# toposware/schnorr-sig

Measured on AMD Instinct MI355X. Metric: Schnorr verifications/sec, 2^20-sig batch, 1/2/4/8 MI355X; bit-exact vs CPU, higher is better.
Workload: dtype u64

## Files before the change

include/schnorr_sig_amd.h:

```cpp
#ifndef SCHNORR_SIG_AMD_H
#define SCHNORR_SIG_AMD_H

#include <stddef.h>
#include <stdint.h>

#ifdef __cplusplus
extern "C" {
#endif

#define SSA_SIGNATURE_LENGTH 81
#define SSA_AFFINE_PK_LENGTH 96
#define SSA_SCALAR_LENGTH 32
#define SSA_PUBLIC_KEY_LENGTH 49
#define SSA_DIGEST_LENGTH 32
#define SSA_PARAMS_LENGTH 2816

#define SSA_OK 0
#define SSA_INVALID_PUBLIC_KEY 1
#define SSA_INVALID_SIGNATURE 2
#define SSA_MALFORMED 3

#define SSA_ERR_ARG (-1)
#define SSA_ERR_HIP (-2)
#define SSA_ERR_PARAMS (-3)
// ... 393 lines not shown
int ssa_aggregator_push(ssa_ctx *ctx, ssa_aggregator *ag, const uint8_t *sigs, const uint8_t *pks, const uint8_t *pk_inf,
                        const uint8_t *msgs, const uint64_t *msg_off, size_t msg_stride, size_t msg_len, size_t n,
                        uint32_t flags, uint8_t *status_out, uint64_t *n_kept_out);
int ssa_aggregator_push_device(ssa_ctx *ctx, ssa_aggregator *ag, const uint8_t *d_sigs, const uint8_t *d_pks,
                               const uint8_t *d_pk_inf, const uint8_t *d_msgs, const uint64_t *d_msg_off, size_t msg_stride,
                               size_t msg_len, size_t n, uint32_t flags, uint8_t *d_status_out, uint64_t *n_kept_out);
int ssa_aggregator_push_cached(ssa_ctx *ctx, ssa_aggregator *ag, ssa_keycache *kc, const uint8_t *sigs, const uint8_t *pks,
                               const uint8_t *pk_inf, const uint8_t *msgs, const uint64_t *msg_off, size_t msg_stride,
                               size_t msg_len, size_t n, uint8_t *status_out, uint64_t *n_kept_out, uint64_t stats_out[12]);
int ssa_aggregator_push_cached_device(ssa_ctx *ctx, ssa_aggregator *ag, ssa_keycache *kc, const uint8_t *d_sigs,
                                      const uint8_t *d_pks, const uint8_t *d_pk_inf, const uint8_t *d_msgs,
                                      const uint64_t *d_msg_off, size_t msg_stride, size_t msg_len, size_t n,
                                      uint8_t *d_status_out, uint64_t *n_kept_out, uint64_t stats_out[12]);
int ssa_aggregator_push_keyed_cached(ssa_ctx *ctx, ssa_aggregator *ag, ssa_keycache *kc, const uint8_t *keyed,
                                     const uint8_t *msgs, const uint64_t *msg_off, size_t msg_stride, size_t msg_len,
                                     size_t n, uint8_t *status_out, uint64_t *n_kept_out, uint64_t stats_out[12]);
int ssa_aggregator_push_keyed_cached_device(ssa_ctx *ctx, ssa_aggregator *ag, ssa_keycache *kc, const uint8_t *d_keyed,
                                            const uint8_t *d_msgs, const uint64_t *d_msg_off, size_t msg_stride,
                                            size_t msg_len, size_t n, uint8_t *d_status_out, uint64_t *n_kept_out,
                                            uint64_t stats_out[12]);
int ssa_aggregator_finish(ssa_ctx *ctx, ssa_aggregator *ag, size_t n_take, uint8_t *agg_out);
int ssa_aggregator_finish_device(ssa_ctx *ctx, ssa_aggregator *ag, size_t n_take, uint8_t *d_agg_out);
int ssa_aggregator_keys(ssa_ctx *ctx, ssa_aggregator *ag, size_t n_take, uint8_t *keys49_out);
int ssa_aggregator_keys_device(ssa_ctx *ctx, ssa_aggregator *ag, size_t n_take, uint8_t *d_keys49_out);
int ssa_debug_aggregator_bytes(size_t capacity, size_t block_lanes, uint32_t flags, uint64_t out[5]);
int ssa_debug_aggregator_plan(uint64_t held, uint64_t m, uint64_t block_lanes, uint64_t out[4]);
int ssa_aggregator_drop_front(ssa_ctx *ctx, ssa_aggregator *ag, size_t n);
int ssa_aggregator_remove(ssa_ctx *ctx, ssa_aggregator *ag, const uint8_t *drop, size_t n_bytes, uint64_t *n_kept_out);
int ssa_aggregator_remove_device(ssa_ctx *ctx, ssa_aggregator *ag, const uint8_t *d_drop, size_t n_bytes,
                                 uint64_t *n_kept_out);
int ssa_aggregator_finish_select(ssa_ctx *ctx, ssa_aggregator *ag, const uint32_t *order, size_t m, uint8_t *agg_out,
                                 uint8_t *keys49_out);
int ssa_aggregator_finish_select_device(ssa_ctx *ctx, ssa_aggregator *ag, const uint32_t *d_order, size_t m,
                                        uint8_t *d_agg_out, uint8_t *d_keys49_out, uint32_t *d_result_out);
int ssa_aggregator_remove_indices(ssa_ctx *ctx, ssa_aggregator *ag, const uint32_t *order, size_t m, uint64_t *n_kept_out);
int ssa_aggregator_remove_indices_device(ssa_ctx *ctx, ssa_aggregator *ag, const uint32_t *d_order, size_t m,
                                         uint64_t *n_kept_out);
int ssa_debug_aggregator_remove_plan(uint64_t held, uint64_t first_changed, uint64_t new_held, uint64_t block_lanes,
                                     uint64_t out[4]);

typedef struct ssa_aggverifier ssa_aggverifier;
int ssa_aggverifier_create(ssa_ctx *ctx, size_t capacity, size_t block_lanes, uint32_t flags, ssa_aggverifier **out);
void ssa_aggverifier_destroy(ssa_aggverifier *av);
int ssa_aggverifier_reset(ssa_aggverifier *av);
int ssa_aggverifier_info(ssa_aggverifier *av, uint64_t out[8]);
int ssa_aggverifier_push(ssa_ctx *ctx, ssa_aggverifier *av, const uint8_t *rs49, const uint8_t *pks, const uint8_t *pk_inf,
                         const uint8_t *msgs, const uint64_t *msg_off, size_t msg_stride, size_t msg_len, size_t n);
int ssa_aggverifier_push_device(ssa_ctx *ctx, ssa_aggverifier *av, const uint8_t *d_rs49, const uint8_t *d_pks,
                                const uint8_t *d_pk_inf, const uint8_t *d_msgs, const uint64_t *d_msg_off,
                                size_t msg_stride, size_t msg_len, size_t n);
int ssa_aggverifier_finish(ssa_ctx *ctx, ssa_aggverifier *av, const uint8_t *e_agg32, size_t n_take);
int ssa_aggverifier_finish_device(ssa_ctx *ctx, ssa_aggverifier *av, const uint8_t *d_e_agg, size_t n_take,
                                  uint32_t *d_verdict_out);
int ssa_debug_aggverifier_record(ssa_ctx *ctx, ssa_aggverifier *av, size_t n_take, uint64_t *d_record24_out);
int ssa_aggverifier_push_cached(ssa_ctx *ctx, ssa_aggverifier *av, ssa_keycache *kc, const uint8_t *rs49, const uint8_t *pks,
                                const uint8_t *pk_inf, const uint8_t *msgs, const uint64_t *msg_off, size_t msg_stride,
                                size_t msg_len, size_t n, uint64_t stats_out[8]);
int ssa_aggverifier_push_cached_device(ssa_ctx *ctx, ssa_aggverifier *av, ssa_keycache *kc, const uint8_t *d_rs49,
                                       const uint8_t *d_pks, const uint8_t *d_pk_inf, const uint8_t *d_msgs,
                                       const uint64_t *d_msg_off, size_t msg_stride, size_t msg_len, size_t n,
                                       uint64_t stats_out[8]);
int ssa_aggverifier_push_cached_wire(ssa_ctx *ctx, ssa_aggverifier *av, ssa_keycache *kc, const uint8_t *rs49,
                                     const uint8_t *pks49, const uint8_t *msgs, const uint64_t *msg_off, size_t msg_stride,
                                     size_t msg_len, size_t n, uint64_t stats_out[8]);
int ssa_aggverifier_push_cached_wire_device(ssa_ctx *ctx, ssa_aggverifier *av, ssa_keycache *kc, const uint8_t *d_rs49,
                                            const uint8_t *d_pks49, const uint8_t *d_msgs, const uint64_t *d_msg_off,
                                            size_t msg_stride, size_t msg_len, size_t n, uint64_t stats_out[8]);
size_t ssa_debug_aggverifier_key_span(void);

#define SSA_ABI_VERSION 5
int ssa_abi_version(void);

int ssa_debug_arith(ssa_ctx *ctx, int op, const uint64_t *a, const uint64_t *b, size_t n,
                    size_t a_stride, size_t b_stride, uint64_t *out, size_t out_stride);
int ssa_debug_fault_after_chunk(ssa_ctx *ctx, int chunk);
int ssa_debug_poison_workspaces(ssa_ctx *ctx, int byte);
int ssa_debug_table_read(ssa_ctx *ctx, int which, uint64_t first_row, uint64_t n, uint64_t *rows_out);
int ssa_debug_table_xor(ssa_ctx *ctx, int which, uint64_t row, uint32_t word, uint64_t mask);
int ssa_debug_corrupt_table_builds(int n);
int ssa_debug_keytab_xor(ssa_keyset *ks, ssa_keycache *kc, int what, uint64_t key, uint32_t word, uint64_t mask);
int ssa_debug_keytab_read(ssa_keyset *ks, ssa_keycache *kc, int what, uint64_t key, uint64_t *words_out);
int ssa_debug_tail_plan(unsigned waves, unsigned pieces, unsigned gens, int uniform, unsigned min_main, size_t n,
                        uint32_t flags, uint32_t out[14]);
int ssa_debug_screen_plan(size_t n, uint32_t coeff_bytes, uint64_t out[8]);
int ssa_debug_screen_segments(ssa_ctx *ctx, uint32_t k);
int ssa_debug_dedup_device(ssa_ctx *ctx, const uint8_t *d_pks, const uint8_t *d_pk_inf, size_t n,
                           uint32_t *d_key_idx_out, uint64_t out[2]);
int ssa_debug_dedup_config(ssa_ctx *ctx, double max_distinct_ratio, uint32_t probe_bound);
int ssa_debug_keycache_plan(uint64_t capacity, uint64_t held, uint64_t u, uint64_t m, uint32_t *plan_out);
int ssa_debug_keycache_keep(uint64_t capacity, uint64_t u, uint64_t m, const uint64_t hist[64], uint64_t out[2]);
int ssa_debug_chacha20(ssa_ctx *ctx, const uint8_t key[32], const uint8_t nonce[12], uint32_t counter0,
                       size_t n_blocks, uint8_t *out);
int ssa_bench_fpmul(ssa_ctx *ctx, int variant, double *fpmul_per_s);

#ifdef __cplusplus
}
#endif
#endif
```

schnorr-sig_amd/__init__.py:

```python
import ctypes as C
import os

import numpy as np

_HERE = os.path.dirname(os.path.abspath(__file__))
LIB_PATH = os.environ.get("SSA_LIB") or os.path.join(_HERE, "csrc", "libschnorr_sig_amd.so")

SCALAR_LENGTH = 32
PRIVATE_KEY_LENGTH = 32
BASEFIELD_LENGTH = 48
PUBLIC_KEY_LENGTH = 49
AFFINE_PUBLIC_KEY_LENGTH = 96
KEY_PAIR_LENGTH = 32
SIGNATURE_LENGTH = 81
KEYED_SIGNATURE_LENGTH = 130

OK, INVALID_PUBLIC_KEY, INVALID_SIGNATURE, MALFORMED = 0, 1, 2, 3
ERR_ARG, ERR_HIP, ERR_PARAMS, ERR_NO_DEVICE, ERR_TABLE = -1, -2, -3, -4, -5
TABLE_COMB, TABLE_CT = 0, 1
SELFCHECK_FIELDS = ("rows", "bad", "first_bad", "ctab_rows", "ctab_bad", "ctab_first_bad", "builds", "bits")
FLAG_CHECK_TORSION = 1
FLAG_FORCE_LANE = 2
FLAG_FORCE_COOP = 4
FLAG_SIG_FLAG_BYTE = 8
# ... 58 lines not shown
        return
    import importlib.util
    spec = importlib.util.find_spec("torch")
    if spec is None or not spec.submodule_search_locations:
        HIP_RUNTIME_BOUND = "system runtime (torch is not installed)"
        return
    path = os.path.join(list(spec.submodule_search_locations)[0], "lib", "libamdhip64.so")
    if not os.path.exists(path):
        HIP_RUNTIME_BOUND = "system runtime (torch carries no libamdhip64.so)"
        return
    try:
        C.CDLL(path, mode=C.RTLD_GLOBAL)
        HIP_RUNTIME_BOUND = path
    except OSError as exc:
        import warnings
        HIP_RUNTIME_BOUND = "system runtime (torch's copy did not load: %s)" % exc
        warnings.warn("schnorr_sig_amd: torch's HIP runtime %s did not load (%s); importing torch later in this process "
                      "will bring a second runtime" % (path, exc))


def _load():
    if not os.path.exists(LIB_PATH):
        raise ImportError(
            "schnorr_sig_amd: HIP library %s is missing; run `python -c 'import __graft_entry__ as g; "
            "g.build()'` (hipcc --offload-arch=gfx950). There is no CPU fallback." % LIB_PATH)
    _share_hip_runtime_with_torch()
    lib = C.CDLL(LIB_PATH)
    vp, sz, u32, u64p, i32 = C.c_void_p, C.c_size_t, C.c_uint32, C.POINTER(C.c_uint64), C.c_int
    sigs = {
        "ssa_ctx_create": (i32, [C.POINTER(vp), i32, vp, sz]),
        "ssa_ctx_create_ex": (i32, [C.POINTER(vp), i32, vp, sz, u32, C.c_uint64]),
        "ssa_ctx_info": (i32, [vp, u64p]),
        "ssa_pubkey_many": (i32, [vp, vp, sz, vp]),
        "ssa_pubkey_many_device": (i32, [vp, vp, sz, vp]),
        "ssa_ctx_destroy": (None, [vp]),
        "ssa_strerror": (C.c_char_p, [i32]),
        "ssa_default_params": (vp, []),
        "ssa_ctx_set_stream": (i32, [vp, vp]),
        "ssa_ctx_uses_default_params": (i32, [vp]),
        "ssa_ctx_sync": (i32, [vp]),
        "ssa_ctx_enable_timing": (i32, [vp, i32]),
        "ssa_ctx_read_timing": (i32, [vp, C.c_char_p, C.POINTER(C.c_double), u64p]),
        "ssa_verify": (i32, [vp, vp, vp, vp, sz, u32]),
        "ssa_verify_many": (i32, [vp, vp, vp, vp, vp, vp, sz, sz, sz, u32, vp, u64p]),
        "ssa_verify_batch": (i32, [vp, vp, vp, vp, vp, vp, sz, sz, sz, u32]),
        "ssa_hash_message_many": (i32, [vp, vp, vp, vp, vp, sz, sz, sz, vp]),
        "ssa_rescue_hash_many": (i32, [vp, vp, u32, sz, vp]),
        "ssa_keygen_sign_many": (i32, [vp, vp, vp, vp, vp, sz, sz, sz, vp, vp]),
        "ssa_verify_many_device": (i32, [vp, vp, vp, vp, vp, vp, sz, sz, sz, u32, vp, vp]),
        "ssa_hash_message_many_device": (i32, [vp, vp, vp, vp, vp, sz, sz, sz, vp]),
        "ssa_rescue_hash_many_device": (i32, [vp, vp, u32, sz, vp]),
        "ssa_keygen_sign_many_device": (i32, [vp, vp, vp, vp, vp, sz, sz, sz, vp, vp]),
        "ssa_verify_batch_msm": (i32, [vp, vp, vp, vp, vp, vp, sz, sz, sz, vp]),
        "ssa_verify_batch_msm_device": (i32, [vp, vp, vp, vp, vp, vp, sz, sz, sz, vp, u32, vp]),
        "ssa_verify_keyed_many": (i32, [vp, vp, vp, vp, sz, sz, sz, u32, vp, u64p]),
        "ssa_keyset_create": (i32, [vp, vp, vp, sz, u32, C.POINTER(vp)]),
        "ssa_keyset_create_device": (i32, [vp, vp, vp, sz, u32, C.POINTER(vp)]),
        "ssa_keyset_destroy": (None, [vp]),
        "ssa_keyset_status": (i32, [vp, vp]),
        "ssa_verify_many_indexed": (i32, [vp, vp, vp, vp, vp, vp, sz, sz, sz, u32, vp, u64p]),
        "ssa_verify_many_indexed_device": (i32, [vp, vp, vp, vp, vp, vp, sz, sz, sz, u32, vp, vp]),
        "ssa_multi_create": (i32, [C.POINTER(vp), C.POINTER(i32), i32, vp, sz]),
        "ssa_multi_destroy": (None, [vp]),
        "ssa_multi_verify_many": (i32, [vp, vp, vp, vp, vp, vp, sz, sz, sz, u32, vp, u64p]),
        "ssa_multi_verify_batch_msm": (i32, [vp, vp, vp, vp, vp, vp, sz, sz, sz, vp]),
        "ssa_decompress_many": (i32, [vp, vp, sz, vp, vp, vp]),
        "ssa_decompress_many_device": (i32, [vp, vp, sz, vp, vp, vp]),
        "ssa_debug_arith": (i32, [vp, i32, vp, vp, sz, sz, sz, vp, sz]),
        "ssa_bench_fpmul": (i32, [vp, i32, C.POINTER(C.c_double)]),
        "ssa_debug_chacha20": (i32, [vp, vp, vp, u32, sz, vp]),
        "ssa_verify_batch_msm_partial_device": (i32, [vp, vp, vp, vp, vp, vp, sz, sz, sz, vp, u32, vp]),
        "ssa_verify_batch_msm_partial": (i32, [vp, vp, vp, vp, vp, vp, sz, sz, sz, vp, vp]),
        "ssa_msm_combine_device": (i32, [vp, vp, sz, vp]),
        "ssa_msm_combine": (i32, [vp, vp, sz]),
        "ssa_abi_version": (i32, []),
        "ssa_keygen_sign_many_ex": (i32, [vp, vp, vp, vp, vp, sz, sz, sz, u32, vp, vp]),
        "ssa_keygen_sign_many_ex_device": (i32, [vp, vp, vp, vp, vp, sz, sz, sz, u32, vp, vp]),
        "ssa_compress_many": (i32, [vp, vp, vp, sz, vp, vp]),
        "ssa_compress_many_device": (i32, [vp, vp, vp, sz, vp, vp]),
        "ssa_ctx_stream_release": (i32, [vp, vp]),
        "ssa_ctx_stream_acquire": (i32, [vp, vp]),
        "ssa_debug_fault_after_chunk": (i32, [vp, i32]),
        "ssa_debug_tail_plan": (i32, [u32, u32, u32, i32, u32, sz, u32, vp]),
        "ssa_verify_batch_screened": (i32, [vp, vp, vp, vp, vp, vp, sz, sz, sz, vp, vp, u64p]),
        "ssa_verify_batch_screened_device": (i32, [vp, vp, vp, vp, vp, vp, sz, sz, sz, vp, u32, vp, vp]),
        "ssa_debug_screen_plan": (i32, [sz, u32, vp]),
        "ssa_debug_screen_segments": (i32, [vp, u32]),
        "ssa_verify_many_dedup": (i32, [vp, vp, vp, vp, vp, vp, sz, sz, sz, u32, vp, u64p, vp]),
        "ssa_verify_many_dedup_device": (i32, [vp, vp, vp, vp, vp, vp, sz, sz, sz, u32, vp, vp, vp]),
        "ssa_verify_many_screened": (i32, [vp, vp, vp, vp, vp, vp, sz, sz, sz, u32, vp, vp, u64p, vp]),
        "ssa_verify_many_screened_device": (i32, [vp, vp, vp, vp, vp, vp, sz, sz, sz, u32, vp, u32, vp, vp, vp]),
        "ssa_keycache_create": (i32, [vp, sz, C.POINTER(vp)]),
        "ssa_keycache_destroy": (None, [vp]),
        "ssa_keycache_clear": (i32, [vp]),
        "ssa_keycache_info": (i32, [vp, u64p]),
        "ssa_verify_many_cached": (i32, [vp, vp, vp, vp, vp, vp, vp, sz, sz, sz, u32, vp, vp, u64p, vp]),
        "ssa_verify_many_cached_device": (i32, [vp, vp, vp, vp, vp, vp, vp, sz, sz, sz, u32, vp, u32, vp, vp, vp]),
        "ssa_keycache_create_ex": (i32, [vp, sz, u32, C.POINTER(vp)]),
        "ssa_verify_keyed_many_cached": (i32, [vp, vp, vp, vp, vp, sz, sz, sz, u32, vp, vp, u64p, vp]),
        "ssa_verify_keyed_many_cached_device": (i32, [vp, vp, vp, vp, vp, sz, sz, sz, u32, vp, u32, vp, vp, vp]),
        "ssa_verify_keyed_many_device": (i32, [vp, vp, vp, vp, sz, sz, sz, u32, vp, vp]),
        "ssa_debug_keycache_plan": (i32, [C.c_uint64, C.c_uint64, C.c_uint64, C.c_uint64, C.POINTER(u32)]),
        "ssa_keycache_set_eviction": (i32, [vp, u32]),
        "ssa_keycache_eviction_info": (i32, [vp, u64p]),
        "ssa_debug_keycache_keep": (i32, [C.c_uint64, C.c_uint64, C.c_uint64, u64p, u64p]),
        "ssa_debug_dedup_device": (i32, [vp, vp, vp, sz, vp, vp]),
        "ssa_debug_dedup_config": (i32, [vp, C.c_double, u32]),
        "ssa_xprv_master_many": (i32, [vp, vp, sz, vp, vp]),
        "ssa_xprv_master_many_device": (i32, [vp, vp, sz, vp, vp]),
        "ssa_xprv_derive_many": (i32, [vp, vp, sz, vp, vp, sz, u32, vp, vp]),
        "ssa_xprv_derive_many_device": (i32, [vp, vp, sz, vp, vp, sz, u32, vp, vp]),
        "ssa_xpub_derive_many": (i32, [vp, vp, sz, vp, vp, sz, vp, vp, vp, vp]),
        "ssa_xpub_derive_many_device": (i32, [vp, vp, sz, vp, vp, sz, vp, vp, vp, vp]),
        "ssa_debug_hmac_sha512": (i32, [vp, vp, sz, vp, sz, sz, vp]),
        "ssa_signer_set_create": (i32, [vp, vp, sz, C.POINTER(vp)]),
        "ssa_signer_set_create_device": (i32, [vp, vp, sz, sz, C.POINTER(vp)]),
        "ssa_signer_set_destroy": (None, [vp]),
        "ssa_signer_set_status": (i32, [vp, vp]),
        "ssa_signer_set_public_keys": (i32, [vp, vp, vp]),
        "ssa_sign_many_indexed": (i32, [vp, vp, vp, vp, vp, vp, sz, sz, sz, u32, vp]),
        "ssa_sign_many_indexed_device": (i32, [vp, vp, vp, vp, vp, vp, sz, sz, sz, u32, vp, vp]),
        "ssa_ctx_selfcheck": (i32, [vp, u32, u64p]),
        "ssa_debug_table_read": (i32, [vp, i32, C.c_uint64, C.c_uint64, vp]),
        "ssa_debug_table_xor": (i32, [vp, i32, C.c_uint64, u32, C.c_uint64]),
        "ssa_debug_corrupt_table_builds": (i32, [i32]),
        "ssa_keyset_selfcheck": (i32, [vp, u32, vp, u64p]),
        "ssa_keycache_selfcheck": (i32, [vp, u32, u64p]),
        "ssa_debug_keytab_xor": (i32, [vp, vp, i32, C.c_uint64, u32, C.c_uint64]),
        "ssa_debug_keytab_read": (i32, [vp, vp, i32, C.c_uint64, vp]),
        "ssa_keygen_sign_many_rng": (i32, [vp, vp, vp, vp, sz, sz, sz, u32, vp, vp]),
        "ssa_keygen_sign_many_rng_device": (i32, [vp, vp, vp, vp, sz, sz, sz, u32, vp, vp]),
        "ssa_sign_many_indexed_rng": (i32, [vp, vp, vp, vp, vp, sz, sz, sz, u32, vp]),
        "ssa_sign_many_indexed_rng_device": (i32, [vp, vp, vp, vp, vp, sz, sz, sz, u32, vp, vp]),
        "ssa_signer_set_generate": (i32, [vp, sz, C.POINTER(vp)]),
        "ssa_signer_set_secret_keys": (i32, [vp, vp]),
        "ssa_debug_pin_rng": (i32, [vp, vp]),
        "ssa_debug_draw_scalars": (i32, [vp, vp, sz, vp]),
        "ssa_debug_poison_workspaces": (i32, [vp, i32]),
        "ssa_aggregate_many": (i32, [vp, vp, vp, vp, vp, vp, sz, sz, sz, u32, vp, vp, u64p]),
        "ssa_aggregate_many_device": (i32, [vp, vp, vp, vp, vp, vp, sz, sz, sz, u32, vp, vp, vp]),
        "ssa_verify_aggregate": (i32, [vp, vp, vp, vp, vp, vp, sz, sz, sz]),
        "ssa_verify_aggregate_device": (i32, [vp, vp, vp, vp, vp, vp, sz, sz, sz, vp]),
        "ssa_debug_aggregate_coeffs": (i32, [vp, vp, vp, vp, vp, vp, sz, sz, sz, vp]),
        "ssa_aggregate_shard_tops_device": (i32, [vp, vp, u32, vp, vp, vp, sz, sz, sz, sz, vp, vp]),
        "ssa_aggregate_root_device": (i32, [vp, vp, sz, sz, sz, vp]),
        "ssa_aggregate_shard_fold_device": (i32, [vp, vp, vp, vp, sz, sz, vp, vp, vp, vp, vp]),
        "ssa_verify_aggregate_shard_device": (i32, [vp, vp, vp, vp, vp, vp, sz, sz, vp, sz, sz, vp, vp]),
        "ssa_aggregate_combine_device": (i32, [vp, vp, sz, vp]),
        "ssa_verify_aggregate_combine_device": (i32, [vp, vp, sz, vp, sz, vp]),
        "ssa_aggregate_many_sliced": (i32, [vp, vp, vp, vp, vp, vp, sz, sz, sz, u32, vp, vp, u64p]),
        "ssa_aggregate_many_sliced_device": (i32, [vp, vp, vp, vp, vp, vp, sz, sz, sz, u32, vp, vp, vp]),
        "ssa_verify_aggregate_sliced": (i32, [vp, vp, vp, vp, vp, vp, sz, sz, sz]),
        "ssa_verify_aggregate_sliced_device": (i32, [vp, vp, vp, vp, vp, vp, sz, sz, sz, vp]),
        "ssa_multi_aggregate_many": (i32, [vp, vp, vp, vp, vp, vp, sz, sz, sz, u32, vp, vp, u64p]),
        "ssa_multi_verify_aggregate": (i32, [vp, vp, vp, vp, vp, vp, sz, sz, sz]),
        "ssa_debug_aggregate_shard_coeffs": (i32, [vp, vp, sz, sz, vp]),
        "ssa_aggregate_valid_many": (i32, [vp, vp, vp, vp, vp, vp, sz, sz, sz, vp, vp, u64p, vp]),
        "ssa_aggregate_valid_many_device": (i32, [vp, vp, vp, vp, vp, vp, sz, sz, sz, vp, vp, u64p, vp]),
        "ssa_aggregate_valid_many_cached": (i32, [vp, vp, vp, vp, vp, vp, vp, sz, sz, sz, vp, vp, u64p, vp, vp, vp, vp]),
        "ssa_aggregate_valid_many_cached_device": (i32, [vp, vp, vp, vp, vp, vp, vp, sz, sz, sz, vp, vp, u64p, vp, vp, vp,
                                                         vp]),
        "ssa_aggregate_valid_keyed_many_cached": (i32, [vp, vp, vp, vp, vp, sz, sz, sz, vp, vp, u64p, vp, vp, vp]),
        "ssa_aggregate_valid_keyed_many_cached_device": (i32, [vp, vp, vp, vp, vp, sz, sz, sz, vp, vp, u64p, vp, vp, vp]),
        "ssa_debug_aggregate_keep": (i32, [vp, vp, sz, vp, u64p]),
        "ssa_verify_aggregates_many": (i32, [vp, vp, u64p, sz, vp, vp, vp, vp, sz, sz, vp]),
        "ssa_verify_aggregates_many_device": (i32, [vp, vp, u64p, sz, vp, vp, vp, vp, sz, sz, vp]),
# ... 1024 lines not shown
        seed = _np_u8(bytearray(seed44))
        if seed.size != 44:
            raise ValueError("the seed is 44 bytes")
        _check(_lib.ssa_debug_pin_rng(self._ctx, _ptr(seed)), "ssa_debug_pin_rng")

    def debug_draw_scalars(self, blocks):
        b = _np_u8(blocks, 128)
        out = np.zeros((b.shape[0], 32), dtype=np.uint8)
        _check(_lib.ssa_debug_draw_scalars(self._ctx, _ptr(b), b.shape[0], _ptr(out)), "ssa_debug_draw_scalars")
        return out

    def set_stream(self, hip_stream):
        _check(_lib.ssa_ctx_set_stream(self._ctx, C.c_void_p(hip_stream or 0)), "ssa_ctx_set_stream")

    def sync(self):
        _check(_lib.ssa_ctx_sync(self._ctx), "ssa_ctx_sync")

    def stream_release(self, consumer_stream):
        _check(_lib.ssa_ctx_stream_release(self._ctx, C.c_void_p(consumer_stream or 0)), "ssa_ctx_stream_release")

    def stream_acquire(self, producer_stream):
        _check(_lib.ssa_ctx_stream_acquire(self._ctx, C.c_void_p(producer_stream or 0)), "ssa_ctx_stream_acquire")

    def selfcheck(self):
        out = (C.c_uint64 * 8)()
        rc = _lib.ssa_ctx_selfcheck(self._ctx, 0, out)
        if rc != ERR_TABLE:
            _check(rc, "ssa_ctx_selfcheck")
        res = dict(zip(SELFCHECK_FIELDS, (int(v) for v in out)))
        res["ok"] = rc == OK
        return res

    def debug_table_read(self, which, first_row, n):
        out = np.zeros((n, 12), dtype=np.uint64)
        _check(_lib.ssa_debug_table_read(self._ctx, int(which), int(first_row), int(n), _ptr(out)), "ssa_debug_table_read")
        return out

    def debug_table_xor(self, which, row, word, mask):
        _check(_lib.ssa_debug_table_xor(self._ctx, int(which), int(row), int(word), C.c_uint64(int(mask))),
               "ssa_debug_table_xor")

    def debug_fault_after_chunk(self, chunk):
        _check(_lib.ssa_debug_fault_after_chunk(self._ctx, int(chunk)), "ssa_debug_fault_after_chunk")

    def debug_poison_workspaces(self, byte):
        _check(_lib.ssa_debug_poison_workspaces(self._ctx, int(byte)), "ssa_debug_poison_workspaces")

    def verify_many_device(self, d_sigs, d_pks, d_msgs, n, msg_len, d_status, d_nfail, msg_stride=None,
                           d_offsets=0, d_pk_inf=0, check_torsion=False, mode=None, sig_flag_byte=False):
        _check(_lib.ssa_verify_many_device(
            self._ctx, d_sigs, d_pks, *self._dev_batch(d_pk_inf, d_msgs, d_offsets, msg_stride, msg_len, n),
            self._verify_flags(check_torsion, sig_flag_byte, mode), d_status, d_nfail), "ssa_verify_many_device")

    def keygen_sign_many_device(self, d_sks, d_nonces, d_msgs, n, msg_len, d_pks, d_sigs, msg_stride=None,
                                d_offsets=0, constant_time=False, keyed=False):
        flags = (FLAG_SIGN_CT if constant_time else 0) | (FLAG_SIGN_KEYED if keyed else 0)
        _check(_lib.ssa_keygen_sign_many_ex_device(self._ctx, d_sks, d_nonces, d_msgs, d_offsets or None,
                                                   msg_stride if msg_stride is not None else msg_len, msg_len, n, flags,
                                                   d_pks or None, d_sigs), "ssa_keygen_sign_many_ex_device")

    def compress_many_device(self, d_pks, n, d_out, d_pk_inf=0, d_status=0):
        _check(_lib.ssa_compress_many_device(self._ctx, d_pks, d_pk_inf or None, n, d_out, d_status or None),
               "ssa_compress_many_device")

    def rescue_hash_many_device(self, d_felts, per_row, n, d_out):
        _check(_lib.ssa_rescue_hash_many_device(self._ctx, d_felts, per_row, n, d_out),
               "ssa_rescue_hash_many_device")

    def hash_message_many_device(self, d_sigs, d_pks, d_msgs, n, msg_len, d_out, msg_stride=None, d_offsets=0):
        _check(_lib.ssa_hash_message_many_device(self._ctx, d_sigs, d_pks, d_msgs, d_offsets or None,
                                                 msg_stride if msg_stride is not None else msg_len, msg_len, n,
                                                 d_out), "ssa_hash_message_many_device")

    def enable_timing(self, on=True):
        _check(_lib.ssa_ctx_enable_timing(self._ctx, int(on)), "ssa_ctx_enable_timing")

    def read_timing(self, kernel):
        avg = C.c_double(0)
        cnt = C.c_uint64(0)
        _check(_lib.ssa_ctx_read_timing(self._ctx, kernel.encode(), C.byref(avg), C.byref(cnt)),
               "ssa_ctx_read_timing")
        return avg.value, int(cnt.value)

    def host_path_probe(self, sigs_t, pks_t, msgs_t, n, reps=3):
        import time
        hs, hp, hm = (t[:n].cpu().numpy() for t in (sigs_t, pks_t, msgs_t))
        st, nf = self.verify_many(hs, hp, hm, check_torsion=False, mode="lane", sig_flag_byte=True)
        t0 = time.perf_counter()
        for _ in range(reps):
            st, nf = self.verify_many(hs, hp, hm, check_torsion=False, mode="lane", sig_flag_byte=True)
        dt = (time.perf_counter() - t0) / reps
        verdict = self.verify_batch_msm(hs, hp, hm)
        t0 = time.perf_counter()
        for _ in range(reps):
            verdict = self.verify_batch_msm(hs, hp, hm)
        dt_msm = (time.perf_counter() - t0) / reps
        return {"entry_point": "ssa_verify_many (host buffers in pageable memory, copied through the library's page-locked "
                               "bounce buffers, uploads in chunks overlapped with the hash kernel)",
                "ms_per_batch": dt * 1e3, "verifications_per_sec": n / dt, "rejected": int(nf),
                "verify_batch_msm_ms_per_batch": dt_msm * 1e3, "verify_batch_msm_signatures_per_sec": n / dt_msm,
                "verify_batch_msm_verdict": int(verdict)}

    def debug_arith(self, op, a, b, out_cols):
        a = np.ascontiguousarray(a, dtype=np.uint64)
        b = np.ascontiguousarray(b, dtype=np.uint64) if b is not None else None
        n = a.shape[0]
        out = np.zeros((n, out_cols), dtype=np.uint64)
        _check(_lib.ssa_debug_arith(self._ctx, op, _ptr(a), _ptr(b), n, a.shape[1],
                                    b.shape[1] if b is not None else 0, _ptr(out), out_cols), "ssa_debug_arith")
        return out

    def bench_fpmul(self, variant):
        v = C.c_double(0)
        _check(_lib.ssa_bench_fpmul(self._ctx, variant, C.byref(v)), "ssa_bench_fpmul")
        return v.value


def debug_corrupt_table_builds(n):
    _check(_lib.ssa_debug_corrupt_table_builds(int(n)), "ssa_debug_corrupt_table_builds")


KEYCHECK_DEEP, KEYCHECK_REPAIR = 1, 2
KEYCHECK_FIELDS = ("keys_checked", "keys_bad", "first_bad_key", "ladder_entries_checked", "comb_rows_checked",
                   "keys_rebuilt_and_compared", "combs_skipped", "rows_repaired")
KEYTAB_LADDER, KEYTAB_STATUS, KEYTAB_KEY, KEYTAB_PK_INF, KEYTAB_COMB = 0, 1, 2, 3, 4
KEYTAB_WIRE = 5
_KEYTAB_READ_WORDS = {KEYTAB_LADDER: 512, KEYTAB_STATUS: 1, KEYTAB_KEY: 12, KEYTAB_PK_INF: 1, KEYTAB_COMB: 24,
                      KEYTAB_WIRE: 7}
KEYCACHE_WIRE = 1
KEYCACHE_EVICT = {"clear": 0, "recent": 1}


def _keycheck_result(rc, out, what):
    if rc != ERR_TABLE:
        _check(rc, what)
    res = dict(zip(KEYCHECK_FIELDS, (int(v) for v in out)))
    res["ok"] = rc == OK
    return res


class _KeyTables:

    def _pair(self):
        raise NotImplementedError

    def debug_keytab_xor(self, what, key, word, mask):
        ks, kc = self._pair()
        _check(_lib.ssa_debug_keytab_xor(ks, kc, int(what), int(key), int(word), C.c_uint64(int(mask))),
               "ssa_debug_keytab_xor")

    def debug_keytab_read(self, what, key):
        ks, kc = self._pair()
        out = np.zeros(_KEYTAB_READ_WORDS[int(what)], dtype=np.uint64)
        _check(_lib.ssa_debug_keytab_read(ks, kc, int(what), int(key), _ptr(out)), "ssa_debug_keytab_read")
        return out


class KeySet(_KeyTables):

    def __init__(self, engine, handle, m):
        self.engine = engine
        self.handle = handle
        self.m = int(m)

    def _pair(self):
        return self.handle, None
# ... 507 lines not shown

class MultiEngine:

    def __init__(self, devices, params=None):
        self._m = C.c_void_p()
        devs = (C.c_int * len(devices))(*[int(d) for d in devices])
        blob = (C.c_uint8 * len(params)).from_buffer_copy(bytes(params)) if params is not None else None
        _check(_lib.ssa_multi_create(C.byref(self._m), devs, len(devices), blob, len(params) if params else 0),
               "ssa_multi_create")

    def close(self):
        if self._m:
            _lib.ssa_multi_destroy(self._m)
            self._m = C.c_void_p()

    def __del__(self):
        try:
            self.close()
        except Exception:
            pass

    def verify_many(self, sigs, pks, msgs, offsets=None, check_torsion=True, pk_inf=None):
        sigs, pks = _np_u8(sigs, 81), _np_u8(pks, 96)
        n = sigs.shape[0]
        m = _np_u8(msgs)
        off = np.ascontiguousarray(offsets, dtype=np.uint64) if offsets is not None else None
        stride = mlen = 0 if off is not None else m.shape[1]
        inf = _np_u8(pk_inf) if pk_inf is not None else None
        status = np.full(n, 255, dtype=np.uint8)
        nfail = C.c_uint64(0)
        _check(_lib.ssa_multi_verify_many(self._m, _ptr(sigs), _ptr(pks), _ptr(inf), _ptr(m), _ptr(off), stride, mlen,
                                          n, FLAG_CHECK_TORSION if check_torsion else 0, _ptr(status),
                                          C.byref(nfail)), "ssa_multi_verify_many")
        return status, int(nfail.value)


    def verify_batch_msm(self, sigs, pks, msgs, offsets=None, coeffs=None, pk_inf=None):
        sigs, pks = _np_u8(sigs, 81), _np_u8(pks, 96)
        n = sigs.shape[0]
        m = _np_u8(msgs)
        off = np.ascontiguousarray(offsets, dtype=np.uint64) if offsets is not None else None
        stride = mlen = 0 if off is not None else m.shape[1]
        inf = _np_u8(pk_inf) if pk_inf is not None else None
        c = _np_u8(coeffs, 32) if coeffs is not None else None
        return _check(_lib.ssa_multi_verify_batch_msm(self._m, _ptr(sigs), _ptr(pks), _ptr(inf), _ptr(m), _ptr(off),
                                                      stride, mlen, n, _ptr(c)), "ssa_multi_verify_batch_msm")


    _msg_args = Engine._msg_args
    _agg_batch = Engine._agg_batch

    def aggregate(self, sigs, pks, msgs, offsets=None, pk_inf=None, check=False):
        n, batch, keep = self._agg_batch(sigs, 81, pks, msgs, offsets, pk_inf)
        agg = np.full(49 * n + 32, 255, dtype=np.uint8)
        status = np.full(n, 255, dtype=np.uint8)
        nfail = C.c_uint64(0)
        st = _check(_lib.ssa_multi_aggregate_many(self._m, *batch, AGG_CHECK if check else 0, _ptr(agg),
                                                  _ptr(status) if n else None, C.byref(nfail)), "ssa_multi_aggregate_many")
        return st, agg, status, int(nfail.value)

    def verify_aggregate(self, agg, pks, msgs, offsets=None, pk_inf=None):
        n, batch, keep = self._agg_batch(agg, 49, pks, msgs, offsets, pk_inf)
        if keep[0].size != 49 * n + 32:
            raise MalformedInput("an aggregate of n signatures is 49 n + 32 bytes")
        return _check(_lib.ssa_multi_verify_aggregate(self._m, *batch), "ssa_multi_verify_aggregate")

    aggregate_sliced, verify_aggregate_sliced = aggregate, verify_aggregate


_default_engine = None


def debug_tail_plan(waves, n, check_torsion=False, pieces=5, gens=1, uniform=False, min_main=0):
    out = np.zeros(14, dtype=np.uint32)
    flags = 1 if check_torsion else 0
    _check(_lib.ssa_debug_tail_plan(int(waves), int(pieces), int(gens), int(bool(uniform)), int(min_main), int(n), flags,
                                    out.ctypes.data), "ssa_debug_tail_plan")

    def dec(d):
        d = int(d)
        return (d & 1, bool(d & 2), bool(d & 4), (d >> 8) & 0xff, (d >> 16) & 0xff)
    return {"n_pieces": int(out[0]), "tail_groups": int(out[1]), "main_blocks": int(out[2]), "grid_blocks": int(out[3]),
            "pieces": [dec(out[4 + k]) for k in range(int(out[0]))], "whole": [dec(out[12]), dec(out[13])]}


def debug_screen_plan(n, coeff_bytes=0):
    out = np.zeros(8, dtype=np.uint64)
    _check(_lib.ssa_debug_screen_plan(int(n), int(coeff_bytes), out.ctypes.data), "ssa_debug_screen_plan")
    keys = ("segments", "segment_lanes", "window_bits", "windows", "r_windows", "buckets_per_window", "slices",
            "total_segments")
    return {k: int(v) for k, v in zip(keys, out)}


def debug_aggregates_plan(counts, msm_slice=1 << 23, small_max=3072):
    counts = np.ascontiguousarray(counts, dtype=np.uint64)
    cp = counts.ctypes.data_as(C.POINTER(C.c_uint64)) if counts.size else None
    need = _lib.ssa_debug_aggregates_plan(cp, counts.size, int(msm_slice), int(small_max), None, 0)
    if need < 0:
        return None
    out = np.zeros(need, dtype=np.uint64)
    _check(_lib.ssa_debug_aggregates_plan(cp, counts.size, int(msm_slice), int(small_max),
                                          out.ctypes.data_as(C.POINTER(C.c_uint64)), need), "ssa_debug_aggregates_plan")
    w = [int(v) for v in out]
    keys = ("first_aggregate", "aggregates", "first_lane", "lanes", "segment_lanes", "bucket")
    groups = [dict(zip(keys, w[4 + 6 * g:10 + 6 * g])) for g in range(w[2])]
    pos, passes = 4 + 6 * w[2], []
    for _ in range(w[1]):
        cnt = w[pos]
        passes.append([tuple(w[pos + 1 + 4 * d:pos + 5 + 4 * d]) for d in range(cnt)])
        pos += 1 + 4 * cnt
    return {"lanes": w[0], "groups": groups, "passes": passes, "descriptors": w[3]}


def debug_aggregates_fold_plan(counts):
    counts = np.ascontiguousarray(counts, dtype=np.uint64)
    cp = counts.ctypes.data_as(C.POINTER(C.c_uint64)) if counts.size else None
    need = _lib.ssa_debug_aggregates_fold_plan(cp, counts.size, None, 0)
    if need < 0:
        return None
    out = np.zeros(need, dtype=np.uint64)
    _check(_lib.ssa_debug_aggregates_fold_plan(cp, counts.size, out.ctypes.data_as(C.POINTER(C.c_uint64)), need),
           "ssa_debug_aggregates_fold_plan")
    return int(out[0]), out[1:]


def default_engine():
    global _default_engine
    if _default_engine is None:
        _default_engine = Engine(0)
    return _default_engine


class PublicKey:

    def __init__(self, affine96, is_identity=False):
        b = bytes(affine96)
        if len(b) != AFFINE_PUBLIC_KEY_LENGTH:
            raise ValueError("PublicKey needs 96 bytes of affine coordinates")
        self.affine = b
        self.is_identity = bool(is_identity)

    def verify_signature(self, signature, message):
        return signature.verify(message, self)

    @classmethod
    def from_private(cls, sk, engine=None):
        return KeyPair.from_private(sk, engine).public_key

    @classmethod
    def from_bytes(cls, b49, engine=None):
        b = bytes(b49)
        if len(b) != PUBLIC_KEY_LENGTH:
            raise ValueError("compressed public key needs 49 bytes")
        pks, inf, st = (engine or default_engine()).decompress_many(np.frombuffer(b, np.uint8))
        if st[0] != 0:
            return None
        return cls(pks[0].tobytes(), is_identity=bool(inf[0]))

    def to_bytes(self, engine=None):
        out, st = (engine or default_engine()).compress_many(np.frombuffer(self.affine, np.uint8),
                                                             pk_inf=np.array([1 if self.is_identity else 0], np.uint8))
        if st[0] != OK:
            raise MalformedInput("PublicKey holds a non-canonical limb")
        return out[0].tobytes()

    def __eq__(self, o):
# ... 544 lines not shown
```

schnorr-sig_amd/csrc/ssa_api.hip:

```cpp
#define SSA_KERNELS_DEFINE 1
#include "ssa_ctx.hpp"
#include "ssa_keycache.hpp"
#include "ssa_keyed.hpp"
#include "ssa_aggregate.hpp"
#include "ssa_aggcache.hpp"
#include "ssa_aggregator.hpp"
#include "ssa_aggverifier.hpp"

#include <sys/random.h>

#include <atomic>
#include <climits>
#include <functional>
#include <initializer_list>
#include <memory>
#include <mutex>
#include <thread>

static const unsigned char k_default_params[SSA_PARAMS_LENGTH] = {
#include "../params/params_default.inc"
};

extern "C" const char *ssa_strerror(int rc) {
    switch (rc) {
        case SSA_OK: return "ok";
        case SSA_INVALID_PUBLIC_KEY: return "The public key is not an element of the prime subgroup.";
        case SSA_INVALID_SIGNATURE: return "The signature is invalid or was incorrectly computed.";
        case SSA_MALFORMED: return "malformed input (the reference would panic)";
        case SSA_ERR_ARG: return "invalid argument";
        case SSA_ERR_HIP: return "HIP runtime error";
        case SSA_ERR_PARAMS: return "invalid parameter blob";
        case SSA_ERR_NO_DEVICE: return "no HIP device";
        case SSA_ERR_TABLE: return "a precomputed table failed its self-check";
        default: return "unknown";
    }
}

extern "C" const void *ssa_default_params(void) { return k_default_params; }

extern "C" int ssa_abi_version(void) { return SSA_ABI_VERSION; }

struct SharedGtab {
    int device = 0;
    u32 bits = 0;
    u64 gen[12] = {};
    u64 *d_gtab = nullptr;
    int refs = 0;
    int builds = 0;
    bool retired = false;
};
static std::mutex g_gtab_mu;
static std::vector<SharedGtab *> g_gtabs;

static inline size_t gtab_bytes(u32 bits) { return gtab_entries(bits) * 12 * sizeof(u64); }

static std::atomic<int> g_corrupt_builds{0};

static int debug_corrupt_build(ssa_ctx *ctx, SharedGtab *g) {
    int n = g_corrupt_builds.load();
    while (n > 0 && !g_corrupt_builds.compare_exchange_weak(n, n - 1)) {
    }
    if (n <= 0) return 0;
    u64 *p = g->d_gtab + 12 * (((size_t)(gtab_windows(g->bits) / 2) << g->bits) + 12345) + 7, v = 0;
    HIP_TRY(hipMemcpyAsync(&v, p, sizeof v, hipMemcpyDeviceToHost, ctx->stream));
    HIP_TRY(hipStreamSynchronize(ctx->stream));
    v ^= 1ull << 17;
    HIP_TRY(hipMemcpyAsync(p, &v, sizeof v, hipMemcpyHostToDevice, ctx->stream));
    HIP_TRY(hipStreamSynchronize(ctx->stream));
    return 0;
}

static SharedGtab *gtab_acquire(ssa_ctx *ctx, const DevParams &hp, u32 bits, bool *bad_table) {
    std::lock_guard<std::mutex> lock(g_gtab_mu);
    u64 gen[12];
    for (int i = 0; i < 6; i++) {
        gen[i] = hp.gen_x[i];
        gen[6 + i] = hp.gen_y[i];
    }
    for (SharedGtab *g : g_gtabs)
        if (g->device == ctx->device && g->bits == bits && std::memcmp(g->gen, gen, sizeof gen) == 0) {
            g->refs++;
            return g;
        }
    SharedGtab *g = new SharedGtab();
    g->device = ctx->device;
    g->bits = bits;
    std::memcpy(g->gen, gen, sizeof gen);
    void *gbase = nullptr;
    bool ok = hipMalloc((void **)&g->d_gtab, gtab_bytes(bits)) == hipSuccess &&
              hipMalloc(&gbase, gbase_entries(bits) * 12 * sizeof(u64)) == hipSuccess;
    if (ok) {
        bool clean = false;
        for (int b = 0; b < 2 && ok && !clean; b++) {
            hipLaunchKernelGGL(ssa_k_gbase, dim3(grid_for(gbase_entries(bits), 256)), dim3(256), 0, ctx->stream,
                               ctx->d_params, (u64 *)gbase, bits);
            hipLaunchKernelGGL(ssa_k_gtable, dim3(grid_for(gtab_entries(bits) / 8, 256)), dim3(256), 0, ctx->stream,
                               (const u64 *)gbase, g->d_gtab, bits);
            g->builds++;
            ok = hipGetLastError() == hipSuccess && hipStreamSynchronize(ctx->stream) == hipSuccess &&
                 debug_corrupt_build(ctx, g) == 0;
            uint64_t res[2] = {0, 0};
            ok = ok && ssa_internal_gtab_check(ctx, g->d_gtab, bits, res) == 0;
            clean = ok && res[0] == 0;
        }
        if (ok && !clean) {
            *bad_table = true;
            ok = false;
        }
    } else {
        (void)hipGetLastError();
    }
    if (gbase) (void)hipFree(gbase);
    if (!ok) {
        if (g->d_gtab) (void)hipFree(g->d_gtab);
        delete g;
        return nullptr;
    }
    g->refs = 1;
    g_gtabs.push_back(g);
    return g;
}

static void gtab_release(SharedGtab *g) {
    if (!g) return;
    std::lock_guard<std::mutex> lock(g_gtab_mu);
    if (--g->refs > 0) return;
    forget_handle(g_gtabs, g);
    (void)hipSetDevice(g->device);
    (void)hipFree(g->d_gtab);
    delete g;
}

static int validate_params(const DevParams &p) {
    if (std::memcmp(p.magic, "SSAPARM1", 8) != 0) return SSA_ERR_PARAMS;
    if (p.n_rounds == 0 || p.n_rounds > 8) return SSA_ERR_PARAMS;
    if (p.rate_off != 0 && p.rate_off != 4) return SSA_ERR_PARAMS;
    if (p.cap_len_idx < -1 || p.cap_len_idx > 11) return SSA_ERR_PARAMS;
    if (p.pad_mode > 1 || p.digest_off > 8) return SSA_ERR_PARAMS;
    for (int i = 0; i < 144; i++)
        if (p.mds[i] >= FP_P) return SSA_ERR_PARAMS;
    for (int i = 0; i < 96; i++)
        if (p.ark1[i] >= FP_P || p.ark2[i] >= FP_P) return SSA_ERR_PARAMS;
    for (int i = 0; i < 6; i++)
        if (p.gen_x[i] >= FP_P || p.gen_y[i] >= FP_P) return SSA_ERR_PARAMS;
    return 0;
}

template <class T>
static bool env_u64(const char *name, uint64_t lo, uint64_t hi, T &knob) {
    const char *e = std::getenv(name);
    const uint64_t v = e ? std::strtoull(e, nullptr, 10) : 0;
    if (!e || v < lo || v > hi) return false;
    knob = (T)v;
    return true;
}
template <class T>
static bool env_int(const char *name, int lo, int hi, T &knob) {
    const char *e = std::getenv(name);
    const int v = e ? std::atoi(e) : 0;
    if (!e || v < lo || v > hi) return false;
    knob = (T)v;
    return true;
}
template <class T>
static void env_one_of(const char *name, std::initializer_list<int> set, T &knob) {
    int v = 0;
    if (env_int(name, INT_MIN, INT_MAX, v) && std::find(set.begin(), set.end(), v) != set.end()) knob = (T)v;
}
static void env_flag(const char *name, bool &knob) {
    int v = 0;
    if (env_int(name, INT_MIN, INT_MAX, v)) knob = v != 0;
}

static void ctx_read_env(ssa_ctx *ctx, uint32_t *gtab_bits, uint64_t *hbm_budget_bytes) {
    CtxKnobs &k = ctx->knobs;
    if (env_u64("SSA_COOP_MAX_N", 0, UINT64_MAX, k.coop_max_n)) k.coop_max_n_torsion = k.coop_max_n;
    env_u64("SSA_MSM_SMALL_MAX", 0, UINT64_MAX, k.msm_small_max);
    env_one_of("SSA_VERIFY_BLOCK", {64, 128, 256}, k.verify_block);
    env_u64("SSA_LANE_SLICE", 256, UINT64_MAX, k.lane_slice);
    env_u64("SSA_MSM_SLICE", 256, (uint64_t)1 << 23, k.msm_slice);
    env_u64("SSA_AGG_BLOCK", 1, (uint64_t)1 << 30, k.agg_block);
    env_int("SSA_MSM_TREE_GROUP", 2, 64, k.msm_tree_group);
    env_int("SSA_TAIL_PIECES", 0, VP_MAX, k.tail_pieces);
    env_int("SSA_TAIL_GENS", 1, 8, k.tail_gens);
    env_flag("SSA_TAIL_UNIFORM", k.tail_uniform);
    env_int("SSA_TAIL_MIN_MAIN", INT_MIN, INT_MAX, k.tail_min_main);
    env_flag("SSA_TAIL_REVERSED", k.tail_reversed);
    env_int("SSA_TAIL_WAVES", INT_MIN, INT_MAX, k.tail_waves_override);
    env_flag("SSA_MSM_OVERLAP", k.msm_overlap);
    env_int("SSA_PIPELINE_CHUNKS", 1, 8, k.pipeline_chunks);
    env_flag("SSA_TWO_STREAMS", ctx->two_streams);
    uint64_t mb = 0;
    if (*hbm_budget_bytes == 0 && env_u64("SSA_HBM_BUDGET_MB", 0, UINT64_MAX, mb)) *hbm_budget_bytes = mb << 20;
    if (*gtab_bits == 0) env_one_of("SSA_GTAB_BITS", {16, 20, 22, 24}, *gtab_bits);
}

static int ctx_create(ssa_ctx **out, int device, const void *params, size_t params_len, uint32_t gtab_bits,
                      uint64_t hbm_budget_bytes, const CtxKnobs *inherit) {
    if (!out) return SSA_ERR_ARG;
    *out = nullptr;
    if (gtab_bits != 0 && gtab_bits != 16 && gtab_bits != 20 && gtab_bits != 22 && gtab_bits != 24) return SSA_ERR_ARG;
    int count = 0;
    if (hipGetDeviceCount(&count) != hipSuccess || count == 0) return SSA_ERR_NO_DEVICE;
    if (device < 0 || device >= count) return SSA_ERR_ARG;
    DevParams hp;
    if (params) {
        if (params_len != sizeof(DevParams)) return SSA_ERR_PARAMS;
        std::memcpy(&hp, params, sizeof hp);
    } else {
        std::memcpy(&hp, k_default_params, sizeof hp);
    }
    const bool is_default = std::memcmp(&hp, k_default_params, sizeof hp) == 0;
    if (int rc = validate_params(hp)) return rc;
    hp.flags = 0;
    bool small_mds = true;
    for (int i = 0; i < 144; i++) small_mds = small_mds && hp.mds[i] <= 0xffffffffull;
    if (small_mds) hp.flags |= PRM_FLAG_SMALL_MDS;
    bool tiny_mds = true;
    for (int i = 0; i < 144; i++) tiny_mds = tiny_mds && hp.mds[i] < 0x10000ull;
    if (tiny_mds) hp.flags |= PRM_FLAG_TINY_MDS;
    HIP_TRY(hipSetDevice(device));
    std::unique_ptr<ssa_ctx, decltype(&ssa_ctx_destroy)> guard(new ssa_ctx(), ssa_ctx_destroy);
    ssa_ctx *ctx = guard.get();
    ctx->device = device;
    ctx->default_params = is_default;
    if (inherit) ctx->knobs = *inherit;
    else ctx_read_env(ctx, &gtab_bits, &hbm_budget_bytes);
    HIP_TRY(hipStreamCreateWithFlags(&ctx->own_stream, hipStreamNonBlocking));
    HIP_TRY(hipStreamCreateWithFlags(&ctx->copy_stream, hipStreamNonBlocking));
    for (auto &st : ctx->hash_stream) HIP_TRY(hipStreamCreateWithFlags(&st, hipStreamNonBlocking));
    HIP_TRY(hipEventCreateWithFlags(&ctx->pipe_start, hipEventDisableTiming));
    HIP_TRY(hipEventCreateWithFlags(&ctx->order_ev, hipEventDisableTiming));
    for (int i = 0; i < 8; i++) {
        HIP_TRY(hipEventCreateWithFlags(&ctx->copy_done[i], hipEventDisableTiming));
        HIP_TRY(hipEventCreateWithFlags(&ctx->hash_done[i], hipEventDisableTiming));
    }
    ctx->stream = ctx->own_stream;
    if (!inherit) {
        hipDeviceProp_t prop;
        int occ = 0;
        if (hipGetDeviceProperties(&prop, device) == hipSuccess &&
            hipOccupancyMaxActiveBlocksPerMultiprocessor(&occ, ssa_k_verify, 256, 0) == hipSuccess && occ > 0)
            ctx->knobs.verify_waves = (unsigned)prop.multiProcessorCount * (unsigned)occ * 4u;
        (void)hipGetLastError();
        if (ctx->knobs.tail_waves_override) ctx->knobs.verify_waves = ctx->knobs.tail_waves_override;
    }
    HIP_TRY(hipMalloc((void **)&ctx->d_params, sizeof(DevParams)));
    HIP_TRY(hipMemcpy(ctx->d_params, &hp, sizeof hp, hipMemcpyHostToDevice));
    ctx->h_params = hp;
    if (hbm_budget_bytes == 0) {
        size_t free_b = 0, total_b = 0;
        if (hipMemGetInfo(&free_b, &total_b) != hipSuccess) free_b = 0;
        hbm_budget_bytes = free_b / 10;
    }
    ctx->hbm_budget = hbm_budget_bytes;
    static const u32 k_widths[4] = {24, 22, 20, 16};
    bool bad_table = false;
    for (u32 wbits : k_widths) {
        if (gtab_bits ? wbits > gtab_bits : (wbits > 16 && gtab_bytes(wbits) > hbm_budget_bytes)) continue;
        ctx->gtab_share = gtab_acquire(ctx, hp, wbits, &bad_table);
        if (ctx->gtab_share) break;
    }
    if (!ctx->gtab_share) return bad_table ? SSA_ERR_TABLE : SSA_ERR_HIP;
    if (ctx->ws_fail.reserve(64)) return SSA_ERR_HIP;
    ctx->d_gtab = ctx->gtab_share->d_gtab;
    ctx->gtab_bits = ctx->gtab_share->bits;
    unsigned gen_ok = 0;
    hipLaunchKernelGGL(ssa_k_check_generator, dim3(1), dim3(64), 0, ctx->stream, ctx->d_params,
                       (const u64 *)ctx->d_gtab, (unsigned *)ctx->ws_fail.p);
    HIP_TRY(hipGetLastError());
    HIP_TRY(hipMemcpyAsync(&gen_ok, ctx->ws_fail.p, sizeof gen_ok, hipMemcpyDeviceToHost, ctx->stream));
    HIP_TRY(hipStreamSynchronize(ctx->stream));
    if (gen_ok != 1u) return SSA_ERR_PARAMS;
    *out = guard.release();
    return 0;
}

extern "C" int ssa_ctx_create_ex(ssa_ctx **out, int device, const void *params, size_t params_len, uint32_t gtab_bits,
                                 uint64_t hbm_budget_bytes) {
    return ctx_create(out, device, params, params_len, gtab_bits, hbm_budget_bytes, nullptr);
}

extern "C" int ssa_ctx_create(ssa_ctx **out, int device, const void *params, size_t params_len) {
    return ssa_ctx_create_ex(out, device, params, params_len, 0u, 0ull);
}

ssa_ctx *ssa_internal_twin(ssa_ctx *ctx) {
    if (ctx->is_twin || !ctx->two_streams) return nullptr;
    if (!ctx->twin) {
        DevParams hp = ctx->h_params;
        hp.flags = 0;
        if (ctx_create(&ctx->twin, ctx->device, &hp, sizeof hp, ctx->gtab_bits, ctx->hbm_budget, &ctx->knobs) != 0) {
            ctx->two_streams = false;
            return nullptr;
        }
        ctx->twin->is_twin = true;
    }
    ctx->twin->knobs = ctx->knobs;
    return ctx->twin;
}

template <class T, class F>
static void orphan_handles(std::vector<T *> &v, F &&release) {
    for (T *h : v) {
        release(h);
        h->ctx = nullptr;
    }
    v.clear();
}

extern "C" void ssa_ctx_destroy(ssa_ctx *ctx) {
    if (!ctx) return;
    (void)hipSetDevice(ctx->device);
    if (ctx->stream) (void)hipStreamSynchronize(ctx->stream);
    if (ctx->twin) {
        ssa_ctx_destroy(ctx->twin);
        ctx->twin = nullptr;
    }
    orphan_handles(ctx->keysets, [](ssa_keyset *ks) { ks->release_all(); });
    orphan_handles(ctx->signer_sets, [](ssa_signer_set *ss) { ss->wipe_release(); });
    orphan_handles(ctx->keycaches, [](ssa_keycache *kc) { kc->release_all(); });
    orphan_handles(ctx->aggregators, [](ssa_aggregator *ag) { agx_release_all(*ag); });
    orphan_handles(ctx->aggverifiers, [](ssa_aggverifier *av) { agx_release_all(*av); });
    for (auto &kv : ctx->timed)
        for (auto &t : kv.second) {
            (void)hipEventDestroy(t.start);
            (void)hipEventDestroy(t.stop);
        }
    for_each_devbuf(ctx, [](DevBuf &b) { b.release(); });
    for_each_hostbuf(ctx, [](HostBuf &b) { b.release(); });
    if (ctx->d_params) (void)hipFree(ctx->d_params);
    gtab_release(ctx->gtab_share);
    ctx->gtab_share = nullptr;
    ctx->d_gtab = nullptr;
    for (auto &ev : ctx->copy_done)
        if (ev) (void)hipEventDestroy(ev);
    for (auto &ev : ctx->hash_done)
        if (ev) (void)hipEventDestroy(ev);
    if (ctx->pipe_start) (void)hipEventDestroy(ctx->pipe_start);
    if (ctx->order_ev) (void)hipEventDestroy(ctx->order_ev);
    if (ctx->agm_plan_ev) (void)hipEventDestroy(ctx->agm_plan_ev);
    for (auto &st : ctx->hash_stream)
        if (st) (void)hipStreamDestroy(st);
    if (ctx->copy_stream) (void)hipStreamDestroy(ctx->copy_stream);
    if (ctx->own_stream) (void)hipStreamDestroy(ctx->own_stream);
    delete ctx;
}

extern "C" int ssa_ctx_info(const ssa_ctx *ctx, uint64_t out[8]) {
    if (!ctx || !out) return SSA_ERR_ARG;
    auto reserved = [](const ssa_ctx *c) {
        uint64_t sum = 0;
        for_each_devbuf(c, [&](const DevBuf &b) { sum += b.cap; });
        return sum;
    };
    out[0] = ctx->gtab_bits;
    out[1] = gtab_windows(ctx->gtab_bits);
    out[2] = gtab_bytes(ctx->gtab_bits);
    out[3] = reserved(ctx) + (ctx->twin ? reserved(ctx->twin) : 0);
    out[4] = ctx->knobs.lane_slice;
    out[5] = ctx->knobs.msm_slice;
    out[6] = ctx->hbm_budget;
    out[7] = ctx->two_streams && !ctx->is_twin ? 1 : 0;
    return 0;
}

extern "C" int ssa_ctx_selfcheck(ssa_ctx *ctx, uint32_t flags, uint64_t out[8]) {
    if (!ctx || !out || flags != 0) return SSA_ERR_ARG;
    HIP_TRY(hipSetDevice(ctx->device));
    uint64_t g[2], c[3] = {0, 0, ~0ull};
    if (int rc = ssa_internal_gtab_check(ctx, ctx->d_gtab, ctx->gtab_bits, g)) return rc;
    if (g[0] == 0)
        if (int rc = ssa_internal_ctab_selfcheck(ctx, c)) return rc;
    out[0] = gtab_entries(ctx->gtab_bits);
    out[1] = g[0];
    out[2] = g[1];
    out[3] = c[0];
    out[4] = c[1];
    out[5] = c[2];
    out[6] = (uint64_t)ctx->gtab_share->builds;
    out[7] = ctx->gtab_bits;
    if (g[0]) {
        std::lock_guard<std::mutex> lock(g_gtab_mu);
        SharedGtab *sg = ctx->gtab_share;
        if (!sg->retired) {
            sg->retired = true;
            forget_handle(g_gtabs, sg);
        }
    }
    return g[0] || c[1] ? SSA_ERR_TABLE : SSA_OK;
}

extern "C" int ssa_ctx_uses_default_params(const ssa_ctx *ctx) { return ctx ? (ctx->default_params ? 1 : 0) : SSA_ERR_ARG; }

extern "C" int ssa_ctx_set_stream(ssa_ctx *ctx, void *hip_stream) {
    if (!ctx) return SSA_ERR_ARG;
    HIP_TRY(hipStreamSynchronize(ctx->stream));
    ctx->stream = hip_stream ? (hipStream_t)hip_stream : ctx->own_stream;
    return 0;
}

extern "C" int ssa_ctx_stream_release(ssa_ctx *ctx, void *consumer_stream) {
    if (!ctx) return SSA_ERR_ARG;
    HIP_TRY(hipSetDevice(ctx->device));
    if ((hipStream_t)consumer_stream == ctx->stream) return 0;
    HIP_TRY(hipEventRecord(ctx->order_ev, ctx->stream));
    HIP_TRY(hipStreamWaitEvent((hipStream_t)consumer_stream, ctx->order_ev, 0));
    return 0;
}

extern "C" int ssa_ctx_stream_acquire(ssa_ctx *ctx, void *producer_stream) {
    if (!ctx) return SSA_ERR_ARG;
    HIP_TRY(hipSetDevice(ctx->device));
    if ((hipStream_t)producer_stream == ctx->stream) return 0;
    HIP_TRY(hipEventRecord(ctx->order_ev, (hipStream_t)producer_stream));
    HIP_TRY(hipStreamWaitEvent(ctx->stream, ctx->order_ev, 0));
    return 0;
}

extern "C" int ssa_ctx_sync(ssa_ctx *ctx) {
    if (!ctx) return SSA_ERR_ARG;
    HIP_TRY(hipStreamSynchronize(ctx->stream));
    return 0;
}

extern "C" int ssa_ctx_enable_timing(ssa_ctx *ctx, int on) {
    if (!ctx) return SSA_ERR_ARG;
    ctx->knobs.timing = on != 0;
    return 0;
}

extern "C" int ssa_ctx_read_timing(ssa_ctx *ctx, const char *kernel, double *avg_ms, uint64_t *launches) {
    if (!ctx || !kernel) return SSA_ERR_ARG;
    HIP_TRY(hipStreamSynchronize(ctx->stream));
    double total = 0;
    uint64_t cnt = 0;
    for (ssa_ctx *c : {ctx, ctx->twin}) {
        if (!c) continue;
        if (c != ctx) HIP_TRY(hipStreamSynchronize(c->stream));
        auto it = c->timed.find(kernel);
        if (it == c->timed.end()) continue;
        for (auto &t : it->second) {
            float ms = 0;
            if (hipEventElapsedTime(&ms, t.start, t.stop) == hipSuccess) {
                total += ms;
                cnt++;
            }
            (void)hipEventDestroy(t.start);
            (void)hipEventDestroy(t.stop);
        }
        c->timed.erase(it);
    }
    if (avg_ms) *avg_ms = cnt ? total / (double)cnt : 0.0;
    if (launches) *launches = cnt;
    return 0;
}

extern "C" int ssa_hash_message_many_device(ssa_ctx *ctx, const uint8_t *d_sigs, const uint8_t *d_pks,
                                            const uint8_t *d_msgs, const uint64_t *d_msg_off,
                                            size_t msg_stride, size_t msg_len, size_t n,
                                            uint8_t *d_digests_out) {
    const MsgView mv{d_msgs, d_msg_off, msg_stride, msg_len};
    if (!ctx || (n && (!d_sigs || !d_pks || !d_digests_out))) return SSA_ERR_ARG;
    if (int rc = check_msgs(mv, n)) return rc;
    if (n == 0) return 0;
    HIP_TRY(hipSetDevice(ctx->device));
    return timed_launch(ctx, "ssa_k_hash", [&] {
        hipLaunchKernelGGL(ssa_k_hash, dim3(grid_for(n, 256)), dim3(256), 0, ctx->stream, ctx->d_params,
                           d_sigs, d_pks, mv, n, (u64 *)nullptr, d_digests_out, (const u32 *)nullptr, 0u);
    });
}

extern "C" int ssa_rescue_hash_many_device(ssa_ctx *ctx, const uint64_t *d_felts, uint32_t felts_per_row,
                                           size_t n, uint64_t *d_digests_out) {
    if (!ctx || (n && (!d_digests_out || (felts_per_row && !d_felts)))) return SSA_ERR_ARG;
    if (n == 0) return 0;
    HIP_TRY(hipSetDevice(ctx->device));
    return timed_launch(ctx, "ssa_k_rescue", [&] {
        hipLaunchKernelGGL(ssa_k_rescue, dim3(grid_for(n, 256)), dim3(256), 0, ctx->stream, ctx->d_params,
                           (const u64 *)d_felts, felts_per_row, n, (u64 *)d_digests_out);
    });
}

int ssa_internal_hash_chunk(ssa_ctx *ctx, hipStream_t hs, const DevBatch &b, size_t cnt, uint64_t *d_h) {
    hipLaunchKernelGGL(ssa_k_hash, dim3(grid_for(cnt, 256)), dim3(256), 0, hs, ctx->d_params, b.sigs, b.pks, b.msgs, cnt,
                       (u64 *)d_h, (u8 *)nullptr, (const u32 *)nullptr, 0u);
    HIP_TRY(hipGetLastError());
    return 0;
}

int ssa_internal_hash_scalars(ssa_ctx *ctx, const DevBatch &b, size_t n) {
    if (ctx->ws_h.reserve(n * 4 * sizeof(u64))) return SSA_ERR_HIP;
    return timed_launch(ctx, "ssa_k_hash", [&] {
        hipLaunchKernelGGL(ssa_k_hash, dim3(grid_for(n, 256)), dim3(256), 0, ctx->stream, ctx->d_params,
                           b.sigs, b.pks, b.msgs, n, (u64 *)ctx->ws_h.p, (u8 *)nullptr, (const u32 *)nullptr, 0u);
    });
}

int ssa_internal_hash_scalars_digests(ssa_ctx *ctx, const DevBatch &b, size_t n, uint64_t *d_h, uint8_t *d_dig) {
    return timed_launch(ctx, "ssa_k_hash", [&] {
        hipLaunchKernelGGL(ssa_k_hash, dim3(grid_for(n, 256)), dim3(256), 0, ctx->stream, ctx->d_params,
                           b.sigs, b.pks, b.msgs, n, (u64 *)d_h, (u8 *)d_dig, (const u32 *)nullptr, 0u);
    });
}

struct TailKnobs {
    unsigned pieces, gens, waves, block, min_main;
    bool uniform, reversed;
};
static TailPlan tail_plan_of(const TailKnobs &kn, size_t cnt, uint32_t flags) {
    const TailKnobs *ctx = &kn;
    TailPlan tp{};
    const bool torsion = (flags & SSA_FLAG_CHECK_TORSION) != 0;
    tp.whole[0] = 0u | 2u | 4u | ((u32)LADDER_STEPS_Q << 16);
    tp.whole[1] = 1u | 2u | 4u | ((u32)LADDER_STEPS << 16);
    const u32 n_groups = (u32)((cnt + 63) / 64);
    const unsigned cap = torsion ? (unsigned)VP_MAX - 1u : (unsigned)VP_MAX;
    const unsigned want = ctx->pieces < cap ? ctx->pieces : cap;
    const u32 tail0 = ctx->gens * ctx->waves;
    if (want < 2 || ctx->block != 256 || tail0 == 0 || n_groups < tail0 + ctx->min_main * ctx->waves) return tp;
    const u32 main_groups = ((n_groups - tail0) / 4u) * 4u;
    tp.main_blocks = main_groups / 4u;
    tp.tail_groups = ((n_groups - main_groups + 3u) / 4u) * 4u;
    const double DBL = 2642.0, ADD = 3738.0, TABLE = 57000.0, TAIL = 45000.0;
    struct Step { int pass, it; double cost; };
    std::vector<Step> steps;
    for (int pass = torsion ? 0 : 1; pass < 2; pass++)
        for (int it = 0; it < (pass == 0 ? LADDER_STEPS_Q : LADDER_STEPS); it++)
            steps.push_back({pass, it, (pass == 0 ? (double)QNAF_GAP[it + 1] : 5.0) * DBL + ADD});
    double total = TABLE + TAIL;
    for (const Step &st : steps) total += st.cost;
    std::vector<double> target;
    double frac = 0.0, f = 0.5;
    for (unsigned k = 0; k + 1 < want; k++) {
        frac += ctx->uniform ? 1.0 / (double)want : f;
        if (k + 2 < want) f *= 0.5;
        target.push_back(total * frac);
    }
    std::vector<std::pair<size_t, size_t>> pieces;
    size_t cur = 0, tix = 0;
    double acc = TABLE;
    for (size_t idx = 0; idx < steps.size(); idx++) {
        bool cut = false;
        if (idx > cur) {
            if (steps[idx].pass != steps[idx - 1].pass) cut = true;
            else if (tix < target.size() && acc + steps[idx].cost * 0.5 >= target[tix]) cut = true;
        }
        if (cut) {
            pieces.push_back({cur, idx});
            cur = idx;
        }
        while (tix < target.size() && acc + steps[idx].cost * 0.5 >= target[tix]) tix++;
        acc += steps[idx].cost;
    }
    pieces.push_back({cur, steps.size()});
    if (pieces.size() < 2 || pieces.size() > (size_t)VP_MAX) return tp;
    for (const auto &pc : pieces) {
        const int pass = steps[pc.first].pass, lo = steps[pc.first].it, hi = steps[pc.second - 1].it + 1;
        const int n_steps = pass == 0 ? LADDER_STEPS_Q : LADDER_STEPS;
        tp.ph[tp.n_pieces++] = (u32)pass | (lo == 0 ? 2u : 0u) | (hi == n_steps ? 4u : 0u) | ((u32)lo << 8) | ((u32)hi << 16);
    }
    tp.reversed = ctx->reversed ? 1u : 0u;
    return tp;
}
static TailPlan tail_plan(const ssa_ctx *ctx, size_t cnt, uint32_t flags) {
    return tail_plan_of({ctx->knobs.tail_pieces, ctx->knobs.tail_gens, ctx->knobs.verify_waves, ctx->knobs.verify_block, ctx->knobs.tail_min_main,
                         ctx->knobs.tail_uniform, ctx->knobs.tail_reversed}, cnt, flags);
}

extern "C" int ssa_debug_tail_plan(unsigned waves, unsigned pieces, unsigned gens, int uniform, unsigned min_main, size_t n,
                                   uint32_t flags, uint32_t out[14]) {
    if (!out) return SSA_ERR_ARG;
    const TailPlan tp = tail_plan_of({pieces, gens, waves, 256u, min_main, uniform != 0, false}, n, flags);
    out[0] = tp.n_pieces;
    out[1] = tp.tail_groups;
    out[2] = tp.main_blocks;
    out[3] = tp.n_pieces ? tail_grid_blocks(tp) : (uint32_t)((n + 255) / 256);
    for (int k = 0; k < VP_MAX; k++) out[4 + k] = tp.ph[k];
    out[12] = tp.whole[0];
    out[13] = tp.whole[1];
    return 0;
}

static int verify_slices(ssa_ctx *ctx, const DevBatch &b, const u64 *d_h, size_t n, uint32_t flags, uint8_t *d_status_out,
                         unsigned long long *d_fail) {
    return for_dev_slices(b, n, ctx->knobs.lane_slice, [&](size_t lo, size_t cnt, const DevBatch &s) {
        const TailPlan tp = tail_plan(ctx, cnt, flags);
        unsigned blocks = grid_for(cnt, ctx->knobs.verify_block);
        if (tp.n_pieces) {
            if (ctx->tail_done.reserve(2 * (size_t)tp.tail_groups * sizeof(u32)) ||
                ctx->tail_park.reserve((size_t)tp.tail_groups * PARK_WORDS * 64 * sizeof(u64)))
                return SSA_ERR_HIP;
            HIP_TRY(hipMemsetAsync(ctx->tail_done.p, 0, 2 * (size_t)tp.tail_groups * sizeof(u32), ctx->stream));
            blocks = tail_grid_blocks(tp);
        }
        return timed_launch(ctx, "ssa_k_verify", [&] {
            hipLaunchKernelGGL(ssa_k_verify, dim3(blocks), dim3(ctx->knobs.verify_block), 0,
                               ctx->stream, s.sigs, s.pks, s.pk_inf, d_h + 4 * lo, (const u64 *)ctx->d_gtab,
                               (u64 *)ctx->ws_tab.p, cnt, flags, d_status_out + lo, d_fail, tp, (u32 *)ctx->tail_done.p,
                               (u64 *)ctx->tail_park.p);
        });
    });
}

int ssa_internal_verify_hashed(ssa_ctx *ctx, const DevBatch &b, const uint64_t *d_h, size_t n, uint32_t flags,
                               uint8_t *d_status_out, unsigned long long *d_fail) {
    const size_t slice = ctx->knobs.lane_slice < n ? ctx->knobs.lane_slice : n;
    if (ctx->ws_tab.reserve(slice * (size_t)(PTAB_ENTRIES * PTAB_ENTRY_U64) * sizeof(u64))) return SSA_ERR_HIP;
    return verify_slices(ctx, b, (const u64 *)d_h, n, flags, d_status_out, d_fail);
}

static int verify_one_slice(ssa_ctx *c, const DevBatch &b, size_t cnt, uint32_t flags, uint8_t *d_status_out,
                            unsigned long long *d_fail) {
    if (c->ws_h.reserve(cnt * 4 * sizeof(u64))) return SSA_ERR_HIP;
    if (c->ws_tab.reserve(cnt * (size_t)(PTAB_ENTRIES * PTAB_ENTRY_U64) * sizeof(u64))) return SSA_ERR_HIP;
    int rc = timed_launch(c, "ssa_k_hash", [&] {
        hipLaunchKernelGGL(ssa_k_hash, dim3(grid_for(cnt, 256)), dim3(256), 0, c->stream, c->d_params, b.sigs, b.pks,
                           b.msgs, cnt, (u64 *)c->ws_h.p, (u8 *)nullptr, (const u32 *)nullptr, 0u);
    });
    if (rc) return rc;
    return verify_slices(c, b, (const u64 *)c->ws_h.p, cnt, flags, d_status_out, d_fail);
}

static int verify_launch(ssa_ctx *ctx, const DevBatch &b, size_t n, uint32_t flags, uint8_t *d_status_out,
                         unsigned long long *d_fail) {
    if (takes_coop(ctx, n, flags)) {
        return timed_launch(ctx, "ssa_k_verify_coop", [&] {
            hipLaunchKernelGGL(ssa_k_verify_coop, dim3((unsigned)n), dim3(128), 0, ctx->stream, ctx->d_params, b.sigs,
                               b.pks, b.pk_inf, b.msgs, (const u64 *)ctx->d_gtab, n, flags, d_status_out, d_fail);
        });
    }
    const size_t slice = ctx->knobs.lane_slice < n ? ctx->knobs.lane_slice : n;
    if (n <= slice) return verify_one_slice(ctx, b, n, flags, d_status_out, d_fail);
    ssa_ctx *tw = ssa_internal_twin(ctx);
    if (tw) {
        HIP_TRY(hipEventRecord(ctx->order_ev, ctx->stream));
        HIP_TRY(hipStreamWaitEvent(tw->stream, ctx->order_ev, 0));
    }
    int rc = 0;
    size_t j = 0;
    for (size_t lo = 0; lo < n && rc == 0; lo += slice, j++) {
        const size_t cnt = n - lo < slice ? n - lo : slice;
        ssa_ctx *c = (tw && (j & 1u)) ? tw : ctx;
        rc = verify_one_slice(c, b.slice(lo), cnt, flags, d_status_out + lo, d_fail);
    }
    if (tw) {
        if (hipEventRecord(tw->order_ev, tw->stream) != hipSuccess ||
            hipStreamWaitEvent(ctx->stream, tw->order_ev, 0) != hipSuccess)
            return rc ? rc : SSA_ERR_HIP;
    }
    return rc;
}

extern "C" int ssa_verify_many_device(ssa_ctx *ctx, const uint8_t *d_sigs, const uint8_t *d_pks,
                                      const uint8_t *d_pk_inf, const uint8_t *d_msgs,
                                      const uint64_t *d_msg_off, size_t msg_stride, size_t msg_len,
                                      size_t n, uint32_t flags, uint8_t *d_status_out,
                                      uint64_t *d_n_fail_out) {
    const DevBatch b{d_sigs, d_pks, d_pk_inf, {d_msgs, d_msg_off, msg_stride, msg_len}};
    if (int rc = check_dev_batch(ctx, b, n, d_status_out)) return rc;
    unsigned long long *d_fail;
    if (int rc = reset_fail_counter(ctx, d_n_fail_out, &d_fail)) return rc;
    if (n == 0) return 0;
    return verify_launch(ctx, b, n, flags, d_status_out, d_fail);
}

int ssa_internal_sign_vartime(ssa_ctx *ctx, const uint8_t *d_sks, const uint8_t *d_nonces, const MsgView &mv, size_t n,
                              uint8_t *d_pks_out, uint8_t *d_sigs_out) {
    return timed_launch(ctx, "ssa_k_sign", [&] {
        hipLaunchKernelGGL(ssa_k_sign, dim3(grid_for(n, 256)), dim3(256), 0, ctx->stream, ctx->d_params,
                           (const u64 *)ctx->d_gtab, d_sks, d_nonces, mv, n, d_pks_out, d_sigs_out);
    });
}

int ssa_internal_sign_indexed_vartime(ssa_ctx *ctx, const ssa_signer_set *ss, const uint32_t *d_key_idx,
                                      const uint8_t *d_nonces, const MsgView &mv, size_t n, bool keyed, uint8_t *d_out,
                                      uint8_t *d_status_out) {
    return timed_launch(ctx, "ssa_k_sign_indexed", [&] {
        hipLaunchKernelGGL(ssa_k_sign_indexed, dim3(grid_for(n, 256)), dim3(256), 0, ctx->stream, ctx->d_params,
                           (const u64 *)ctx->d_gtab, ss->view(), d_key_idx, d_nonces, mv, n, keyed ? 1u : 0u, d_out,
                           d_status_out);
    });
}

extern "C" int ssa_keygen_sign_many_device(ssa_ctx *ctx, const uint8_t *d_sks, const uint8_t *d_nonces,
                                           const uint8_t *d_msgs, const uint64_t *d_msg_off,
                                           size_t msg_stride, size_t msg_len, size_t n,
                                           uint8_t *d_pks_out, uint8_t *d_sigs_out) {
    return ssa_keygen_sign_many_ex_device(ctx, d_sks, d_nonces, d_msgs, d_msg_off, msg_stride, msg_len, n, 0u, d_pks_out,
                                          d_sigs_out);
}

extern "C" int ssa_decompress_many_device(ssa_ctx *ctx, const uint8_t *d_compressed, size_t n,
                                          uint8_t *d_pks_out, uint8_t *d_pk_inf_out, uint8_t *d_status_out) {
    if (!ctx || (n && (!d_compressed || !d_pks_out || !d_status_out)) || n > SSA_MAX_BATCH) return SSA_ERR_ARG;
    if (n == 0) return 0;
    HIP_TRY(hipSetDevice(ctx->device));
    return timed_launch(ctx, "ssa_k_decompress", [&] {
        hipLaunchKernelGGL(ssa_k_decompress, dim3(grid_for(n, 256)), dim3(256), 0, ctx->stream, d_compressed, n,
                           d_pks_out, d_pk_inf_out, d_status_out);
    });
}

static int verify_many_host_one(ssa_ctx *ctx, const HostBatch &b, size_t n, uint32_t flags, uint8_t *status_out,
                                uint64_t *n_fail_out) {
    return status_host_one(ctx, b, n, nullptr, !takes_coop(ctx, n, flags), true, status_out, n_fail_out,
                           [&](const StagedInputs &s, u8 *d_status, unsigned long long *d_fail) {
        HIP_TRY(hipMemsetAsync(d_fail, 0, sizeof(unsigned long long), ctx->stream));
        if (!s.hashed) return verify_launch(ctx, s.batch, n, flags, d_status, d_fail);
        return ssa_internal_verify_hashed(ctx, s.batch, (const uint64_t *)ctx->ws_h.p, n, flags, d_status, d_fail);
    });
}

extern "C" int ssa_verify_many(ssa_ctx *ctx, const uint8_t *sigs, const uint8_t *pks, const uint8_t *pk_inf,
                               const uint8_t *msgs, const uint64_t *msg_off, size_t msg_stride,
                               size_t msg_len, size_t n, uint32_t flags, uint8_t *status_out,
                               uint64_t *n_fail_out) {
    const HostBatch b{sigs, pks, pk_inf, msgs, msg_off, msg_stride, msg_len};
    if (int rc = check_host_batch(ctx, b, n, status_out)) return rc;
    if (n_fail_out) *n_fail_out = 0;
    if (n == 0) return 0;
    HIP_TRY(hipSetDevice(ctx->device));
    return run_host_slices_counted(ctx, b, n, ctx->knobs.lane_slice, n_fail_out,
                                   [&](ssa_ctx *c, size_t lo, size_t cnt, const HostBatch &s, uint64_t *nf) {
                                       return verify_many_host_one(c, s, cnt, flags, status_out + lo, nf);
                                   });
}

extern "C" int ssa_verify_batch(ssa_ctx *ctx, const uint8_t *sigs, const uint8_t *pks, const uint8_t *pk_inf,
                                const uint8_t *msgs, const uint64_t *msg_off, size_t msg_stride, size_t msg_len,
                                size_t n, uint32_t flags) {
    if (n == 0) return ctx ? SSA_OK : SSA_ERR_ARG;
    std::vector<uint8_t> status(n);
    uint64_t nf = 0;
    if (int rc = ssa_verify_many(ctx, sigs, pks, pk_inf, msgs, msg_off, msg_stride, msg_len, n,
                                 flags | SSA_FLAG_SIG_FLAG_BYTE, status.data(), &nf))
        return rc;
    if (nf == 0) return SSA_OK;
    bool any_pk = false;
    for (uint8_t s : status) {
        if (s == SSA_MALFORMED) return SSA_MALFORMED;
        any_pk = any_pk || s == SSA_INVALID_PUBLIC_KEY;
    }
    return any_pk ? SSA_INVALID_PUBLIC_KEY : SSA_INVALID_SIGNATURE;
}

extern "C" int ssa_verify(ssa_ctx *ctx, const uint8_t sig[SSA_SIGNATURE_LENGTH],
                          const uint8_t pk[SSA_AFFINE_PK_LENGTH], const uint8_t *msg, size_t msg_len,
                          uint32_t flags) {
    uint8_t st = SSA_MALFORMED;
    if (int rc = ssa_verify_many(ctx, sig, pk, nullptr, msg, nullptr, msg_len, msg_len, 1, flags, &st, nullptr))
        return rc;
    return st;
}

extern "C" int ssa_hash_message_many(ssa_ctx *ctx, const uint8_t *sigs, const uint8_t *pks, const uint8_t *msgs,
                                     const uint64_t *msg_off, size_t msg_stride, size_t msg_len, size_t n,
                                     uint8_t *digests_out) {
    if (!ctx || (n && (!sigs || !pks || !digests_out))) return SSA_ERR_ARG;
    if (int rc = check_msgs({msgs, msg_off, msg_stride, msg_len}, n)) return rc;
    if (int rc = check_host_offsets(msg_off, n)) return rc;
    if (n == 0) return 0;
    HostCall hc(ctx);
    const u8 *d_sigs = hc.in(ctx->st_sigs, sigs, n * 81), *d_pks = hc.in(ctx->st_pks, pks, n * 96);
    const MsgView mv = hc.msgs(msgs, msg_off, msg_stride, msg_len, n);
    u8 *d_out = hc.out(ctx->st_aux, digests_out, n * 32);
    return hc.finish([&] {
        return ssa_hash_message_many_device(ctx, d_sigs, d_pks, mv.msgs, mv.off, msg_stride, msg_len, n, d_out);
    });
}

extern "C" int ssa_rescue_hash_many(ssa_ctx *ctx, const uint64_t *felts, uint32_t felts_per_row, size_t n,
                                    uint64_t *digests_out) {
    if (!ctx || (n && (!digests_out || (felts_per_row && !felts)))) return SSA_ERR_ARG;
    if (n == 0) return 0;
    HostCall hc(ctx);
    const uint64_t *d_felts = hc.in<uint64_t>(ctx->st_aux, felts, n * (size_t)felts_per_row * 8);
    u8 *d_out = hc.out(ctx->st_aux2, digests_out, n * 32);
    return hc.finish([&] { return ssa_rescue_hash_many_device(ctx, d_felts, felts_per_row, n, (uint64_t *)d_out); });
}

extern "C" int ssa_keygen_sign_many(ssa_ctx *ctx, const uint8_t *sks, const uint8_t *nonces,
                                    const uint8_t *msgs, const uint64_t *msg_off, size_t msg_stride,
                                    size_t msg_len, size_t n, uint8_t *pks_out, uint8_t *sigs_out) {
    if (n && !pks_out) return SSA_ERR_ARG;
    return ssa_keygen_sign_many_ex(ctx, sks, nonces, msgs, msg_off, msg_stride, msg_len, n, 0u, pks_out, sigs_out);
}

extern "C" int ssa_decompress_many(ssa_ctx *ctx, const uint8_t *compressed, size_t n, uint8_t *pks_out,
                                   uint8_t *pk_inf_out, uint8_t *status_out) {
    if (!ctx || (n && (!compressed || !pks_out || !status_out))) return SSA_ERR_ARG;
    if (n == 0) return 0;
    HostCall hc(ctx);
    const u8 *d_in = hc.in(ctx->st_sigs, compressed, n * 49);
    u8 *d_pks = hc.out(ctx->st_aux, pks_out, n * 96), *d_inf = hc.out(ctx->st_aux2, pk_inf_out, n, 16),
       *d_status = hc.out(ctx->st_status, status_out, n, 16);
    return hc.finish([&] { return ssa_decompress_many_device(ctx, d_in, n, d_pks, d_inf, d_status); });
}

static int verify_keyed_host_one(ssa_ctx *ctx, const uint8_t *keyed, const HostBatch &b, size_t n, uint32_t flags,
                                 uint8_t *status_out, uint64_t *n_fail_out) {
    HostCall hc(ctx);
    const u8 *d_keyed = hc.in(ctx->st_keyed, keyed, n * 130);
    u8 *d_sigs = hc.out(ctx->st_sigs, nullptr, n * 81), *d_pks = hc.out(ctx->st_pks, nullptr, n * 96),
       *d_inf = hc.out(ctx->st_inf, nullptr, n, 16), *d_status = hc.out(ctx->st_status, status_out, n, 16);
    hc.step([&] {
        hipLaunchKernelGGL(ssa_k_unpack_keyed, dim3(grid_for(n, 256)), dim3(256), 0, ctx->stream, d_keyed, n, d_pks, d_inf,
                           d_sigs);
        HIP_TRY(hipGetLastError());
        return 0;
    });
    const MsgView mv = hc.msgs(b.msgs, b.msg_off, b.msg_stride, b.msg_len, n);
    unsigned long long nf = 0, *d_fail = (unsigned long long *)ctx->ws_fail.p;
    hc.copy_back(&nf, d_fail, sizeof nf);
    if (int rc = hc.finish([&] {
            return ssa_verify_many_device(ctx, d_sigs, d_pks, d_inf, mv.msgs, mv.off, b.msg_stride, b.msg_len, n, flags,
                                          d_status, (uint64_t *)d_fail);
        }))
        return rc;
    if (n_fail_out) *n_fail_out = nf;
    return 0;
}

extern "C" int ssa_verify_keyed_many(ssa_ctx *ctx, const uint8_t *keyed, const uint8_t *msgs,
                                     const uint64_t *msg_off, size_t msg_stride, size_t msg_len, size_t n,
                                     uint32_t flags, uint8_t *status_out, uint64_t *n_fail_out) {
    if (!ctx || (n && (!keyed || !status_out))) return SSA_ERR_ARG;
    if (int rc = check_msgs({msgs, msg_off, msg_stride, msg_len}, n)) return rc;
    if (int rc = check_host_offsets(msg_off, n)) return rc;
    if (n_fail_out) *n_fail_out = 0;
    if (n == 0) return 0;
    HIP_TRY(hipSetDevice(ctx->device));
    const HostBatch b{nullptr, nullptr, nullptr, msgs, msg_off, msg_stride, msg_len};
    return run_host_slices_counted(ctx, b, n, ctx->knobs.lane_slice, n_fail_out,
                                   [&](ssa_ctx *c, size_t lo, size_t cnt, const HostBatch &s, uint64_t *nf) {
                                       return verify_keyed_host_one(c, keyed + 130 * lo, s, cnt, flags, status_out + lo, nf);
                                   });
}


int ssa_internal_keyset_build(ssa_ctx *ctx, const uint8_t *d_pks, const uint8_t *d_pk_inf, size_t m, uint64_t *d_tab,
                              uint8_t *d_status) {
    return timed_launch(ctx, "ssa_k_keyset_build", [&] {
        hipLaunchKernelGGL(ssa_k_keyset_build, dim3(grid_for(m, 256)), dim3(256), 0, ctx->stream, d_pks, d_pk_inf, m,
                           (u64 *)d_tab, d_status);
    });
}

extern "C" int ssa_keyset_create_device(ssa_ctx *ctx, const uint8_t *d_pks, const uint8_t *d_pk_inf, size_t m,
                                        uint32_t flags, ssa_keyset **out) {
    if (!ctx || !out || !d_pks || m == 0 || m > 0xffffffffull || flags > SSA_KEYSET_LADDER) return SSA_ERR_ARG;
    *out = nullptr;
    HIP_TRY(hipSetDevice(ctx->device));
    std::unique_ptr<ssa_keyset, decltype(&ssa_keyset_destroy)> guard(new ssa_keyset(), ssa_keyset_destroy);
    ssa_keyset *ks = guard.get();
    ks->ctx = ctx;
    ks->m = m;
    if (ks->tab.reserve(m * (size_t)(PTAB_ENTRIES * PTAB_ENTRY_U64) * sizeof(u64)) || ks->status.reserve(m + 16) ||
        ks->pks.reserve(m * 96) || ks->inf.reserve(m + 16))
        return SSA_ERR_HIP;
    HIP_TRY(hipMemcpyAsync(ks->pks.p, d_pks, m * 96, hipMemcpyDeviceToDevice, ctx->stream));
    HIP_TRY(d_pk_inf ? hipMemcpyAsync(ks->inf.p, d_pk_inf, m, hipMemcpyDeviceToDevice, ctx->stream)
                     : hipMemsetAsync(ks->inf.p, 0, m, ctx->stream));
    if (int rc = ssa_internal_keyset_build(ctx, (const u8 *)ks->pks.p, (const u8 *)ks->inf.p, m, (u64 *)ks->tab.p,
                                           (u8 *)ks->status.p))
        return rc;
    HIP_TRY(hipStreamSynchronize(ctx->stream));
    const size_t comb_bytes = m * KTAB_ENTRIES_PER_KEY * 12 * sizeof(u64);
    const size_t comb_cap = ctx->hbm_budget < ((uint64_t)16 << 30) ? (size_t)ctx->hbm_budget : ((size_t)16 << 30);
    ks->comb = flags == SSA_KEYSET_COMB || (flags == SSA_KEYSET_AUTO && comb_bytes <= comb_cap);
    DevBuf kbase;
    if (ks->comb && (ks->ktab.reserve(comb_bytes) || kbase.reserve(m * KBASE_ENTRIES_PER_KEY * 12 * sizeof(u64)))) {
        kbase.release();
        ks->ktab.release();
        (void)hipGetLastError();
        if (flags == SSA_KEYSET_COMB) return SSA_ERR_HIP;
        ks->comb = false;
    }
    if (ks->comb) {
        const int rc = timed_launch(ctx, "ssa_k_keycomb_build", [&] {
            hipLaunchKernelGGL(ssa_k_keycomb_base, dim3(grid_for(m * KBASE_ENTRIES_PER_KEY, 256)), dim3(256), 0,
                               ctx->stream, (const u8 *)ks->pks.p, (const u8 *)ks->inf.p, (const u8 *)ks->status.p, m,
                               (u64 *)kbase.p);
            hipLaunchKernelGGL(ssa_k_keycomb_build, dim3(grid_for(m * (KTAB_ENTRIES_PER_KEY / 8), 256)), dim3(256), 0,
                               ctx->stream, (const u64 *)kbase.p, m, (u64 *)ks->ktab.p);
        });
        const bool synced = hipStreamSynchronize(ctx->stream) == hipSuccess;
        kbase.release();
        if (rc != 0 || !synced) return rc ? rc : SSA_ERR_HIP;
    }
    ctx->keysets.push_back(ks);
    *out = guard.release();
    return 0;
}

extern "C" int ssa_keyset_create(ssa_ctx *ctx, const uint8_t *pks, const uint8_t *pk_inf, size_t m, uint32_t flags,
                                 ssa_keyset **out) {
    if (!ctx || !out || !pks || m == 0) return SSA_ERR_ARG;
    HostCall hc(ctx);
    const u8 *d_pks = hc.in(ctx->st_pks, pks, m * 96), *d_inf = pk_inf ? hc.in(ctx->st_inf, pk_inf, m) : nullptr;
// ... 3091 lines not shown
```

schnorr-sig_amd/csrc/ssa_ctx.hpp:

```cpp
#pragma once
#include "../../include/schnorr_sig_amd.h"
#include "ssa_kernels.hpp"

#include <hip/hip_runtime.h>

#include <algorithm>
#include <cstdio>
#include <cstdlib>
#include <cstring>
#include <functional>
#include <map>
#include <mutex>
#include <string>
#include <thread>
#include <utility>
#include <vector>

using namespace ssa;

static inline bool ssa_debug_enabled() {
    static const bool on = std::getenv("SSA_DEBUG") != nullptr;
    return on;
}
#define HIP_TRY(expr)                                                                    \
    do {                                                                                 \
        hipError_t err__ = (expr);                                                       \
        if (err__ != hipSuccess) {                                                       \
            if (ssa_debug_enabled())                                                     \
                std::fprintf(stderr, "[schnorr_sig_amd] %s failed: %s (%s:%d)\n", #expr, \
                             hipGetErrorString(err__), __FILE__, __LINE__);              \
            return SSA_ERR_HIP;                                                          \
        }                                                                                \
    } while (0)

struct DevBuf {
    void *p = nullptr;
    size_t cap = 0;
    int reserve(size_t bytes) {
        if (bytes <= cap) return 0;
        if (p) (void)hipFree(p);
        p = nullptr;
        cap = 0;
        size_t want = bytes + bytes / 8 + 256;
        if (hipMalloc(&p, want) != hipSuccess) return SSA_ERR_HIP;
        cap = want;
        return 0;
    }
    int reserve_exact(size_t bytes) {
        release();
        const size_t want = (bytes + 255) & ~(size_t)255;
        if (hipMalloc(&p, want) != hipSuccess) {
            p = nullptr;
            return SSA_ERR_HIP;
        }
        cap = want;
        return 0;
    }
    void release() {
        if (p) (void)hipFree(p);
        p = nullptr;
        cap = 0;
    }
};

struct HostBuf {
    void *p = nullptr;
    size_t cap = 0;
    int reserve(size_t bytes) {
        if (bytes <= cap) return 0;
        if (p) (void)hipHostFree(p);
        p = nullptr;
        cap = 0;
        const size_t want = bytes + bytes / 8 + 4096;
        if (hipHostMalloc(&p, want, hipHostMallocDefault) != hipSuccess) {
            (void)hipGetLastError();
            p = nullptr;
            return SSA_ERR_HIP;
        }
        cap = want;
        return 0;
    }
    void release() {
        if (p) (void)hipHostFree(p);
        p = nullptr;
        cap = 0;
    }
};

struct TimedLaunch {
    hipEvent_t start, stop;
};

constexpr double DEDUP_RATIO_NO_CHECK = 0.0, DEDUP_RATIO_CHECK = 1.0;
constexpr unsigned DEDUP_PROBE_BOUND = 128;

struct CtxKnobs {
    size_t pipeline_min_n = 1 << 17;
    unsigned pipeline_chunks = 8;
    size_t coop_max_n = 7680, coop_max_n_torsion = 10496;
    size_t msm_small_max = 3072;
    size_t lane_slice = (size_t)1 << 20, msm_slice = (size_t)1 << 23;
    size_t agg_block = 0;
    bool msm_overlap = true;
    unsigned msm_tree_group = 16;
    unsigned verify_block = 256;
    unsigned verify_waves = 0;
    unsigned tail_pieces = 5;
    unsigned tail_gens = 1;
    bool tail_uniform = false;
    bool tail_reversed = false;
    unsigned tail_min_main = 0;
    unsigned tail_waves_override = 0;
    bool timing = false;
    unsigned screen_segs = 0;
    double dedup_ratio[2] = {DEDUP_RATIO_NO_CHECK, DEDUP_RATIO_CHECK};
    unsigned dedup_probe_bound = DEDUP_PROBE_BOUND;
};

#define SSA_CTX_DEVBUFS(X) \
    X(ws_h) X(ws_tab) X(ws_fail) \
     \
    X(st_sigs) X(st_pks) X(st_inf) X(st_msgs) X(st_off) X(st_status) X(st_aux) X(st_aux2) X(st_coeffs) \
     \
    X(msm_points) X(msm_scalars) X(msm_keys) X(msm_vals) X(msm_keys2) X(msm_vals2) X(msm_sort_tmp) X(msm_bounds) \
    X(msm_buckets) X(msm_chunks) X(msm_windows) X(msm_partials) X(msm_flags) X(msm_cnt) X(msm_cnt2) X(msm_ids) \
    X(msm_ids2) X(msm_comb_pts) X(msm_comb_lins) \
    X(msm_slice_recs)    \
    X(msm_sbuf)          \
     \
    X(scr_ok) X(scr_in) X(scr_status) X(scr_fail) \
     \
    X(scr_mask) X(scr_mark) X(scr_list) X(scr_blk) X(scr_cnt) \
     \
    X(dd_slots) X(dd_rep) X(dd_num) X(dd_reps) X(dd_idx) X(dd_blk) X(dd_stats) X(dd_pks) X(dd_inf) X(dd_kstatus) \
     \
    X(kc_found) X(kc_missrep) X(kc_blk) X(kc_lane_row) \
     \
    X(st_keyed) X(ky_sigs) X(ky_pks) X(ky_inf) \
     \
    X(ctab) X(sg_sigs) X(sg_pks) \
    X(tc_out)            \
    X(kck_ws)            \
    X(dv_recs)           \
     \
    X(rng_seed) X(rng_scratch) \
     \
    X(ag_sigs) X(ag_dig) X(ag_nodes) X(ag_nodes2) X(ag_coeffs) X(ag_partials) X(ag_status) X(ag_misc) \
     \
    X(agm_plan) X(agm_map) X(agm_roots) X(agm_in) X(agm_bytes) \
     \
    X(agp_acc) \
     \
    X(av_blk) X(av_sigs) X(av_dig) \
     \
    X(avc_keys) X(avc_inf) \
     \
    X(agc_kst) X(agc_pks) X(agc_inf) X(agc_cnt) \
     \
    X(ags_tops) X(ags_parts) X(ags_recs) \
     \
    X(agx_kept) \
     \
    X(agx_stage) X(agx_first) \
     \
    X(agx_sel_stage) X(agx_sel_bits) X(agx_sel_order) X(agx_sel_mask) \
     \
    X(tail_done) X(tail_park)

#define SSA_CTX_HOSTBUFS(X) X(pin_in) X(pin_coeffs) X(pin_out) X(pin_seed)

struct ssa_ctx {
    int device = 0;
    hipStream_t own_stream = nullptr;
    hipStream_t stream = nullptr;
    hipStream_t copy_stream = nullptr;
    hipEvent_t copy_done[8] = {};
    hipStream_t hash_stream[2] = {};
    hipEvent_t hash_done[8] = {};
    hipEvent_t pipe_start = nullptr;
    hipEvent_t order_ev = nullptr;
    hipEvent_t agm_plan_ev = nullptr;
    std::vector<uint32_t> agm_plan_host;
    CtxKnobs knobs;
    DevParams *d_params = nullptr;
    u64 *d_gtab = nullptr;
    struct SharedGtab *gtab_share = nullptr;
    uint32_t gtab_bits = 0;
    uint64_t hbm_budget = 0;
    DevParams h_params;
    ssa_ctx *twin = nullptr;
    bool is_twin = false, two_streams = true;
#define X(name) DevBuf name;
    SSA_CTX_DEVBUFS(X)
#undef X
#define X(name) HostBuf name;
    SSA_CTX_HOSTBUFS(X)
#undef X
    bool default_params = false;
    int fault_after_chunk = -1;
    uint64_t dedup_key[2] = {0, 0};
    bool dedup_key_set = false;
    bool ctab_ready = false;
    bool rng_pinned = false;
    uint8_t rng_pin[44] = {};
    std::map<std::string, std::vector<TimedLaunch>> timed;
    std::vector<struct ssa_keyset *> keysets;
    std::vector<struct ssa_signer_set *> signer_sets;
    std::vector<struct ssa_keycache *> keycaches;
    std::vector<struct ssa_aggregator *> aggregators;
    std::vector<struct ssa_aggverifier *> aggverifiers;
};

template <class Ctx, class F>
static inline void for_each_devbuf(Ctx *c, F &&f) {
#define X(name) f(c->name);
    SSA_CTX_DEVBUFS(X)
#undef X
}
template <class Ctx, class F>
static inline void for_each_hostbuf(Ctx *c, F &&f) {
#define X(name) f(c->name);
    SSA_CTX_HOSTBUFS(X)
#undef X
}

template <class T>
static inline void forget_handle(std::vector<T *> &v, T *p) {
    const auto it = std::find(v.begin(), v.end(), p);
    if (it != v.end()) v.erase(it);
}

struct ssa_keyset {
    ssa_ctx *ctx = nullptr;
    size_t m = 0;
    bool comb = false;
    DevBuf tab, status, pks, inf, ktab;
    void release_all() {
        tab.release();
        status.release();
        pks.release();
        inf.release();
        ktab.release();
    }
};

struct ssa_keycache {
    ssa_ctx *ctx = nullptr;
    size_t capacity = 0, held = 0, n_slots = 0;
    uint64_t clears = 0;
    bool wire_mode = false;
    ssa_keyset rows;
    DevBuf inf, slots, wire;
    uint32_t policy = 0;
    uint64_t epoch = 0, compactions = 0, dropped = 0, last_kept = 0, last_moved = 0;
    DevBuf stamps, evict_ws;
    uint64_t device_bytes() const {
        return rows.tab.cap + rows.status.cap + rows.pks.cap + inf.cap + slots.cap + wire.cap + stamps.cap + evict_ws.cap;
    }
    void release_all() {
        rows.release_all();
        inf.release();
        slots.release();
        wire.release();
        stamps.release();
        evict_ws.release();
    }
};

struct ssa_signer_set {
    ssa_ctx *ctx = nullptr;
    size_t m = 0;
    DevBuf sks, pks, cpks, status;
    std::vector<uint8_t> host_status;
    SignerView view() const { return {(const u8 *)sks.p, (const u8 *)pks.p, (const u8 *)cpks.p, (const u8 *)status.p, (u32)m}; }
    void wipe_release() {
        if (sks.p) {
            (void)hipMemsetAsync(sks.p, 0, sks.cap, ctx->stream);
            (void)hipStreamSynchronize(ctx->stream);
        }
        sks.release();
        pks.release();
        cpks.release();
        status.release();
    }
};

static inline unsigned grid_for(size_t n, unsigned block) { return (unsigned)((n + block - 1) / block); }

template <class F>
static inline int timed_launch(ssa_ctx *ctx, const char *name, F &&launch) {
    if (!ctx->knobs.timing) {
        launch();
        HIP_TRY(hipGetLastError());
        return 0;
    }
    TimedLaunch t;
    HIP_TRY(hipEventCreate(&t.start));
    HIP_TRY(hipEventCreate(&t.stop));
    HIP_TRY(hipEventRecord(t.start, ctx->stream));
    launch();
    HIP_TRY(hipGetLastError());
    HIP_TRY(hipEventRecord(t.stop, ctx->stream));
    ctx->timed[name].push_back(t);
    return 0;
}


static inline int check_msgs(const MsgView &mv, size_t n) {
    if (n == 0) return 0;
    if (n > SSA_MAX_BATCH) return SSA_ERR_ARG;
    if (!mv.off && mv.len > 0 && !mv.msgs) return SSA_ERR_ARG;
    if (!mv.off && mv.stride < mv.len) return SSA_ERR_ARG;
    if (mv.len > 0xffffffffull) return SSA_ERR_ARG;
    return 0;
}

static inline int check_host_offsets(const uint64_t *off, size_t n) {
    if (off)
        for (size_t i = 0; i < n; i++)
            if (off[i + 1] < off[i] || off[i + 1] - off[i] > 0xffffffffull) return SSA_ERR_ARG;
    return 0;
}

static inline size_t msgs_bytes(const uint64_t *off, size_t stride, size_t len, size_t n) {
    if (n == 0) return 0;
    if (off) return (size_t)off[n];
    return (n - 1) * stride + len;
}

struct HostBatch {
    const uint8_t *sigs, *pks, *pk_inf, *msgs;
    const uint64_t *msg_off;
    size_t msg_stride, msg_len;
    HostBatch slice(size_t lo, size_t cnt, std::vector<uint64_t> &off) const {
        HostBatch s = *this;
        s.sigs = sigs ? sigs + 81 * lo : nullptr;
        s.pks = pks ? pks + 96 * lo : nullptr;
        s.pk_inf = pk_inf ? pk_inf + lo : nullptr;
        if (msg_off) {
            off.resize(cnt + 1);
            for (size_t k = 0; k <= cnt; k++) off[k] = msg_off[lo + k] - msg_off[lo];
            s.msgs = msgs ? msgs + msg_off[lo] : nullptr;
            s.msg_off = off.data();
        } else {
            s.msgs = msgs ? msgs + lo * msg_stride : nullptr;
        }
        return s;
    }
};

struct DevBatch {
    const uint8_t *sigs, *pks, *pk_inf;
    MsgView msgs;
    DevBatch slice(size_t lo) const {
        DevBatch s = *this;
        s.sigs = sigs ? sigs + 81 * lo : nullptr;
        s.pks = pks ? pks + 96 * lo : nullptr;
        s.pk_inf = pk_inf ? pk_inf + lo : nullptr;
        if (msgs.off) s.msgs.off = msgs.off + lo;
        else if (msgs.msgs) s.msgs.msgs = msgs.msgs + lo * msgs.stride;
        return s;
    }
};

template <class F>
static inline int for_dev_slices(const DevBatch &b, size_t n, size_t slice, F &&fn) {
    for (size_t lo = 0; lo < n; lo += slice)
        if (int rc = fn(lo, n - lo < slice ? n - lo : slice, b.slice(lo))) return rc;
    return 0;
}

static inline int check_host_batch(const ssa_ctx *ctx, const HostBatch &b, size_t n, const uint8_t *status_out) {
    if (!ctx || (n && (!b.sigs || !b.pks || !status_out))) return SSA_ERR_ARG;
    if (int rc = check_msgs({b.msgs, b.msg_off, b.msg_stride, b.msg_len}, n)) return rc;
    return check_host_offsets(b.msg_off, n);
}
static inline int check_dev_batch(const ssa_ctx *ctx, const DevBatch &b, size_t n, const uint8_t *d_status_out,
                                  const uint8_t *d_coeffs = nullptr, uint32_t coeff_bytes = 32) {
    if (!ctx || (n && (!b.sigs || !b.pks || !d_status_out))) return SSA_ERR_ARG;
    if (d_coeffs && (coeff_bytes == 0 || coeff_bytes > 32)) return SSA_ERR_ARG;
    return check_msgs(b.msgs, n);
}

static inline bool takes_coop(const ssa_ctx *ctx, size_t n, uint32_t flags) {
    const size_t coop_lim = (flags & SSA_FLAG_CHECK_TORSION) ? ctx->knobs.coop_max_n_torsion : ctx->knobs.coop_max_n;
    return (flags & SSA_FLAG_FORCE_COOP) || (!(flags & SSA_FLAG_FORCE_LANE) && n <= coop_lim);
}

struct CallStats {
    const int width;
    std::mutex mu;
    uint64_t v[12] = {0, 0, 0, 0, 0, 0, 0, 0, 0, 0, 0, 0};
    explicit CallStats(int words) : width(words) {}
    void add(const uint64_t *d) {
        std::lock_guard<std::mutex> lock(mu);
        for (int k = 0; k < width; k++) v[k] += d[k];
    }
    void out(uint64_t *stats_out) const {
        if (stats_out)
            for (int k = 0; k < width; k++) stats_out[k] = v[k];
    }
};

struct StagedInputs {
    DevBatch batch{};
    const u8 *coeffs = nullptr;
    bool hashed = false;
};

static inline int reset_fail_counter(ssa_ctx *ctx, uint64_t *d_n_fail_out, unsigned long long **d_fail) {
    HIP_TRY(hipSetDevice(ctx->device));
    *d_fail = (unsigned long long *)(d_n_fail_out ? (void *)d_n_fail_out : ctx->ws_fail.p);
    HIP_TRY(hipMemsetAsync(*d_fail, 0, sizeof(unsigned long long), ctx->stream));
    return 0;
}

struct SecretWipe {
    ssa_ctx *ctx;
    std::vector<std::pair<DevBuf *, size_t>> bufs;
    void add(DevBuf &b, size_t bytes) { bufs.emplace_back(&b, bytes); }
    bool zero() {
        bool any = false;
        for (auto &b : bufs)
            if (b.first->p && b.second) {
                (void)hipMemsetAsync(b.first->p, 0, std::min(b.second, b.first->cap), ctx->stream);
                any = true;
            }
        bufs.clear();
        return any;
    }
    ~SecretWipe() { zero(); }
};

constexpr bool SECRET = true;

struct HostCall {
    ssa_ctx *ctx;
    int rc = 0;
    bool enqueued = false, settled = false;
    SecretWipe wipe{ctx};
    struct Back { void *dst; const void *src; size_t bytes; };
    std::vector<Back> back;

    explicit HostCall(ssa_ctx *c) : ctx(c) { hip(hipSetDevice(ctx->device)); }
    ~HostCall() {
        const bool zeroed = wipe.zero();
        if (zeroed || (enqueued && !settled)) (void)hipStreamSynchronize(ctx->stream);
    }
    bool ok() const { return rc == 0; }
    void hip(hipError_t err) {
        if (err == hipSuccess || rc) return;
        if (ssa_debug_enabled()) std::fprintf(stderr, "[schnorr_sig_amd] host call: %s\n", hipGetErrorString(err));
        rc = SSA_ERR_HIP;
    }
    template <class F>
    void step(F &&f) {
        if (rc) return;
        enqueued = true;
        rc = f();
    }
    template <class T = u8>
    const T *in(DevBuf &buf, const void *src, size_t bytes, bool secret = false) {
        if (rc) return nullptr;
        if (secret) wipe.add(buf, bytes);
        enqueued = true;
        if (buf.reserve(src && bytes ? bytes : 16)) rc = SSA_ERR_HIP;
        else if (src && bytes) hip(hipMemcpyAsync(buf.p, src, bytes, hipMemcpyHostToDevice, ctx->stream));
        return rc || !src ? nullptr : (const T *)buf.p;
    }
// ... 158 lines not shown
        else hc.rc = pipelined_upload_hash(ctx, b, n, pin, &used);
        if (!hc.ok() || used) {
            StagedInputs s = pin.s;
            s.hashed = true;
            if (coeffs && hc.ok()) {
                host_copy(ctx->pin_coeffs.p, coeffs, n * 32);
                hc.step([&] {
                    HIP_TRY(hipMemcpyAsync(ctx->st_coeffs.p, ctx->pin_coeffs.p, n * 32, hipMemcpyHostToDevice, ctx->copy_stream));
                    HIP_TRY(hipEventRecord(ctx->pipe_start, ctx->copy_stream));
                    HIP_TRY(hipStreamWaitEvent(ctx->stream, ctx->pipe_start, 0));
                    return 0;
                });
                s.coeffs = (const u8 *)ctx->st_coeffs.p;
            }
            return s;
        }
    }
    StagedInputs s;
    s.batch.sigs = hc.in(ctx->st_sigs, b.sigs, n * 81);
    s.batch.pks = hc.in(ctx->st_pks, b.pks, n * 96);
    if (b.pk_inf) s.batch.pk_inf = hc.in(ctx->st_inf, b.pk_inf, n);
    s.batch.msgs = hc.msgs(b.msgs, b.msg_off, b.msg_stride, b.msg_len, n);
    if (coeffs) s.coeffs = hc.in(ctx->st_coeffs, coeffs, n * 32);
    return s;
}

template <class F>
static int status_host_one(ssa_ctx *ctx, const HostBatch &b, size_t n, const uint8_t *coeffs, bool pipeline, bool pin_out,
                           uint8_t *status_out, uint64_t *n_fail_out, F &&device_form) {
    HostCall hc(ctx);
    PipelinedInputs pin;
    const StagedInputs s = slice_inputs(hc, pin, b, n, coeffs, pipeline, pin_out);
    const bool through_pin = pin_out && s.hashed;
    u8 *d_status = hc.out(ctx->st_status, through_pin ? ctx->pin_out.p : status_out, n, 16);
    unsigned long long nf = 0, *d_fail = (unsigned long long *)ctx->ws_fail.p;
    hc.copy_back(&nf, d_fail, sizeof nf);
    if (int rc = hc.finish([&] { return device_form(s, d_status, d_fail); })) return rc;
    pin.done();
    if (through_pin) std::memcpy(status_out, ctx->pin_out.p, n);
    if (n_fail_out) *n_fail_out = nf;
    return 0;
}

int ssa_internal_hash_scalars(ssa_ctx *ctx, const DevBatch &b, size_t n);

int ssa_internal_hash_scalars_digests(ssa_ctx *ctx, const DevBatch &b, size_t n, uint64_t *d_h, uint8_t *d_dig);

int ssa_internal_msm_record(ssa_ctx *ctx, const DevBatch &b, size_t n, const uint8_t *d_coeffs, uint32_t coeff_bytes,
                            const uint64_t *d_h, uint64_t *d_record_out);

struct MsmFill {
    MsmShape sh;
    u32 wa;
    size_t n;
    unsigned n_blocks;
    u64 *points;
    short *digits;
    u64 *partials;
    u32 *flags;
};
using MsmFillFn = std::function<int(const MsmFill &)>;
int ssa_internal_msm_record_prepared(ssa_ctx *ctx, size_t n, uint32_t coeff_bytes, const MsmFillFn &fill,
                                     uint64_t *d_record_out);

int ssa_internal_msm_sum_records(ssa_ctx *ctx, const uint64_t *d_records, size_t k, bool checked, uint64_t *d_record_out);

int ssa_internal_msm_agg_small(ssa_ctx *ctx, const DevBatch &b, size_t n, const uint8_t *d_coeffs16, const uint32_t *d_first,
                               uint32_t agg0, uint32_t aggs, const uint64_t **d_recs_out);
int ssa_internal_msm_agg_segments(ssa_ctx *ctx, const DevBatch &b, uint32_t segs, uint32_t seg_lanes,
                                  const uint8_t *d_coeffs16, const uint64_t *d_h, const uint8_t *d_mask, uint8_t *d_recheck,
                                  const uint8_t *d_rhs, uint8_t *d_seg_ok);

int ssa_internal_screen_hashed(ssa_ctx *ctx, const DevBatch &b, size_t n, const uint64_t *d_h, uint8_t *d_status,
                               unsigned long long *d_fail);

int ssa_internal_screen_many_hashed(ssa_ctx *ctx, struct ssa_keycache *kc, const DevBatch &b, size_t n, const uint64_t *d_h,
                                    uint8_t *d_status, uint64_t stats_out[12]);
int ssa_internal_screen_keyed_hashed(ssa_ctx *ctx, struct ssa_keycache *kc, const uint8_t *d_keyed, const MsgView &mv,
                                     size_t n, uint64_t *d_h, uint8_t *d_dig, uint8_t *d_status, uint64_t stats_out[12]);

int ssa_internal_verify_hashed(ssa_ctx *ctx, const DevBatch &b, const uint64_t *d_h, size_t n, uint32_t flags,
                               uint8_t *d_status_out, unsigned long long *d_fail);

int ssa_internal_dedup_keys(ssa_ctx *ctx, const uint8_t *d_pks, const uint8_t *d_pk_inf, size_t cnt, uint64_t *u_out,
                            uint64_t *bound_hits_out);
int ssa_internal_verify_keyed(ssa_ctx *ctx, const uint8_t *d_sigs, const uint32_t *d_key_idx, uint64_t u,
                              const uint64_t *d_h, size_t n, uint32_t flags, uint8_t *d_status_out,
                              unsigned long long *d_fail);

struct KeyView {
    const uint32_t *lane_key;
    const uint64_t *tab;
    const uint8_t *status;
    uint32_t n_keys;
};
static inline KeyView ctx_key_view(const ssa_ctx *ctx, uint64_t u) {
    return {(const uint32_t *)ctx->dd_idx.p, (const uint64_t *)ctx->ws_tab.p, (const uint8_t *)ctx->dd_kstatus.p, (uint32_t)u};
}
int ssa_internal_verify_keyed_view(ssa_ctx *ctx, const uint8_t *d_sigs, const uint32_t *d_lane_key, const KeyView &kv,
                                   const uint64_t *d_h, size_t n, uint32_t flags, uint8_t *d_status_out,
                                   unsigned long long *d_fail);

int ssa_internal_keycache_slice(ssa_ctx *ctx, struct ssa_keycache *kc, const uint8_t *d_pks, const uint8_t *d_pk_inf,
                                size_t cnt, KeyView *kv, uint64_t *u_out, uint64_t *bound_hits_out, uint64_t ks[4],
                                const unsigned long long **d_unpublished);

int ssa_internal_keyed_cache_slice(ssa_ctx *ctx, struct ssa_keycache *kc, const uint8_t *d_keyed, size_t cnt, DevBatch *b,
                                   KeyView *kv, uint64_t *u_out, uint64_t *bound_hits_out, uint64_t ks[4],
                                   const unsigned long long **d_unpublished);
int ssa_internal_unpack_keyed(ssa_ctx *ctx, const uint8_t *d_keyed, size_t n, DevBatch *b);

int ssa_internal_keyset_build(ssa_ctx *ctx, const uint8_t *d_pks, const uint8_t *d_pk_inf, size_t m, uint64_t *d_tab,
                              uint8_t *d_status);

int ssa_internal_gtab_check(ssa_ctx *ctx, const uint64_t *d_gtab, uint32_t bits, uint64_t res[2]);
int ssa_internal_ctab_selfcheck(ssa_ctx *ctx, uint64_t out[3]);

ssa_ctx *ssa_internal_twin(ssa_ctx *ctx);

template <class F>
static int run_host_slices(ssa_ctx *ctx, size_t n, size_t slice, F &&fn) {
    const size_t k = (n + slice - 1) / slice;
    ssa_ctx *tw = k > 1 ? ssa_internal_twin(ctx) : nullptr;
    if (!tw) {
        for (size_t j = 0; j < k; j++) {
            const size_t lo = j * slice, cnt = n - lo < slice ? n - lo : slice;
            if (int rc = fn(ctx, lo, cnt)) return rc;
        }
        return 0;
    }
    int rcs[2] = {0, 0};
    auto worker = [&](size_t w) {
        if (hipSetDevice(ctx->device) != hipSuccess) {
            rcs[w] = SSA_ERR_HIP;
            return;
        }
        ssa_ctx *c = w ? tw : ctx;
        for (size_t j = w; j < k && rcs[w] == 0; j += 2) {
            const size_t lo = j * slice, cnt = n - lo < slice ? n - lo : slice;
            rcs[w] = fn(c, lo, cnt);
        }
    };
    std::thread second(worker, (size_t)1);
    worker(0);
    second.join();
    return rcs[0] ? rcs[0] : rcs[1];
}

template <class F>
static int run_host_slices_counted(ssa_ctx *ctx, const HostBatch &b, size_t n, size_t slice, uint64_t *n_fail_out, F &&fn) {
    if (n <= slice) return fn(ctx, (size_t)0, n, b, n_fail_out);
    std::mutex mu;
    uint64_t total = 0;
    const int rc = run_host_slices(ctx, n, slice, [&](ssa_ctx *c, size_t lo, size_t cnt) {
        std::vector<uint64_t> off;
        uint64_t nf = 0;
        const int r = fn(c, lo, cnt, b.slice(lo, cnt, off), &nf);
        std::lock_guard<std::mutex> lock(mu);
        total += nf;
        return r;
    });
    if (rc) return rc;
    if (n_fail_out) *n_fail_out = total;
    return 0;
}
```

schnorr-sig_amd/csrc/ssa_msm.hip:

```cpp
#define SSA_NO_KERNELS 1
#include "ssa_ctx.hpp"

#include <sys/random.h>

namespace ssa {

constexpr int MSM_CHUNK = 8;

constexpr u32 MSM_TILE = 16384;
constexpr u32 MSM_HI_BINS = 256;
constexpr u32 MSM_LO_BITS = 7, MSM_LO_BINS = 1u << MSM_LO_BITS;
constexpr u32 MSM_MAX_WINDOWS = 32;

struct MsmItems {
    u32 n, wa, windows;
    u32 seg_blocks, cm1;
    u32 tile0[MSM_MAX_WINDOWS + 1];
    u32 base[MSM_MAX_WINDOWS + 1];
};
SSA_DEV u32 items_of_window(const MsmItems &it, u32 j) { return j < it.wa ? 2u * it.n : it.n; }
SSA_DEV u32 item_point(const MsmItems &it, u32 j, u32 k) { return j < it.wa ? k : it.n + k; }


__global__ void __launch_bounds__(256)
// ... 1331 lines not shown
    return 0;
}

extern "C" int ssa_verify_batch_msm_partial(ssa_ctx *ctx, const uint8_t *sigs, const uint8_t *pks, const uint8_t *pk_inf,
                                            const uint8_t *msgs, const uint64_t *msg_off, size_t msg_stride,
                                            size_t msg_len, size_t n, const uint8_t *coeffs,
                                            uint64_t out24[SSA_MSM_PARTIAL_WORDS]) {
    if (!ctx || !out24 || (n && (!sigs || !pks))) return SSA_ERR_ARG;
    if (int rc = check_msgs({msgs, msg_off, msg_stride, msg_len}, n)) return rc;
    HIP_TRY(hipSetDevice(ctx->device));
    std::memset(out24, 0, SSA_MSM_PARTIAL_WORDS * sizeof(uint64_t));
    if (n == 0) {
        out24[23] = SSA_MSM_RECORD_MAGIC;
        return 0;
    }
    if (int rc = check_host_offsets(msg_off, n)) return rc;
    const HostBatch b{sigs, pks, pk_inf, msgs, msg_off, msg_stride, msg_len};
    return n > ctx->knobs.msm_slice ? msm_host_sliced(ctx, b, n, coeffs, nullptr, out24)
                              : msm_host_one(ctx, b, n, coeffs, nullptr, out24);
}

extern "C" int ssa_verify_batch_msm(ssa_ctx *ctx, const uint8_t *sigs, const uint8_t *pks, const uint8_t *pk_inf,
                                    const uint8_t *msgs, const uint64_t *msg_off, size_t msg_stride, size_t msg_len,
                                    size_t n, const uint8_t *coeffs) {
    if (!ctx || (n && (!sigs || !pks))) return SSA_ERR_ARG;
    if (int rc = check_msgs({msgs, msg_off, msg_stride, msg_len}, n)) return rc;
    if (int rc = check_host_offsets(msg_off, n)) return rc;
    if (n == 0) return SSA_OK;
    HIP_TRY(hipSetDevice(ctx->device));
    const HostBatch b{sigs, pks, pk_inf, msgs, msg_off, msg_stride, msg_len};
    int verdict = SSA_MALFORMED;
    const int rc = n > ctx->knobs.msm_slice ? msm_host_sliced(ctx, b, n, coeffs, &verdict, nullptr)
                                      : msm_host_one(ctx, b, n, coeffs, &verdict, nullptr);
    return rc ? rc : verdict;
}

constexpr u32 SCREEN_MAX_SEGS = 256;
constexpr u32 SCREEN_MIN_SEG_LANES = 1024;

struct ScreenPlan {
    u32 segs, seg_lanes;
};
static ScreenPlan screen_plan(size_t n, unsigned forced) {
    size_t k = forced;
    if (k == 0) {
        k = SCREEN_MAX_SEGS;
        while (k > 1 && n / k < SCREEN_MIN_SEG_LANES) k >>= 1;
    }
    size_t per = (n + k - 1) / k;
    per = (per + 255) & ~(size_t)255;
    return {(u32)((n + per - 1) / per), (u32)per};
}

extern "C" int ssa_debug_screen_plan(size_t n, uint32_t coeff_bytes, uint64_t out[8]) {
    if (!out || n == 0 || n > SSA_MAX_BATCH || coeff_bytes > 32) return SSA_ERR_ARG;
    const size_t slice = (size_t)1 << 23;
    const size_t first = n < slice ? n : slice, slices = (n + slice - 1) / slice, last = n - (slices - 1) * slice;
    const ScreenPlan pl = screen_plan(first, 0);
    const MsmShape sh = screen_shape(pl.segs);
    const u32 cb = coeff_bytes ? coeff_bytes : 16u;
    out[0] = pl.segs;
    out[1] = pl.seg_lanes;
    out[2] = sh.c;
    out[3] = sh.windows;
    out[4] = cb >= 32 ? sh.windows : (8u * cb + sh.c - 1) / sh.c;
    out[5] = sh.buckets;
    out[6] = slices;
    out[7] = (uint64_t)(slices - 1) * pl.segs + screen_plan(last, 0).segs;
    return 0;
}

extern "C" int ssa_debug_screen_segments(ssa_ctx *ctx, uint32_t k) {
    if (!ctx || k > SCREEN_MAX_SEGS) return SSA_ERR_ARG;
    ctx->knobs.screen_segs = k;
    return 0;
}

static int screen_slice(ssa_ctx *ctx, const DevBatch &b, size_t n, const uint8_t *d_coeffs, uint32_t coeff_bytes,
                        const u64 *d_h, uint8_t *d_status) {
    if (ctx->scr_fail.reserve(16)) return SSA_ERR_HIP;
    unsigned long long *scratch_fail = (unsigned long long *)ctx->scr_fail.p;
    if (n <= ctx->knobs.msm_small_max) {
        if (d_h) return ssa_internal_verify_hashed(ctx, b, d_h, n, SSA_FLAG_SIG_FLAG_BYTE, d_status, scratch_fail);
        return ssa_verify_many_device(ctx, b.sigs, b.pks, b.pk_inf, b.msgs.msgs, b.msgs.off, b.msgs.stride, b.msgs.len, n,
                                      SSA_FLAG_SIG_FLAG_BYTE, d_status, (uint64_t *)scratch_fail);
    }
    const ScreenPlan pl = screen_plan(n, ctx->knobs.screen_segs);
    if (ctx->scr_ok.reserve(SCREEN_MAX_SEGS)) return SSA_ERR_HIP;
    const ScreenArgs sa{pl.segs, pl.seg_lanes / 256u, d_status, (u8 *)ctx->scr_ok.p};
    if (int rc = msm_run_one(ctx, b, n, d_coeffs, coeff_bytes, nullptr, nullptr, d_h, &sa)) return rc;
    const u64 *h = d_h ? d_h : (const u64 *)ctx->ws_h.p;
    uint8_t ok[SCREEN_MAX_SEGS];
    HIP_TRY(hipMemcpyAsync(ok, ctx->scr_ok.p, pl.segs, hipMemcpyDeviceToHost, ctx->stream));
    HIP_TRY(hipStreamSynchronize(ctx->stream));
    ScreenList sl{};
    sl.seg_lanes = pl.seg_lanes;
    sl.n = (u32)n;
    size_t m = 0;
    for (u32 s = 0; s < pl.segs; s++) {
        if (ok[s]) continue;
        sl.id[sl.count++] = (uint16_t)s;
        const size_t lo = (size_t)s * pl.seg_lanes;
        m += n - lo < pl.seg_lanes ? n - lo : pl.seg_lanes;
    }
    if (m == 0) return 0;
    if (2 * m > n)
        return ssa_internal_verify_hashed(ctx, b, h, n, SSA_FLAG_SIG_FLAG_BYTE, d_status, scratch_fail);
    auto al = [](size_t b) { return (b + 255) & ~(size_t)255; };
    const size_t o_pks = al(m * 81), o_h = o_pks + al(m * 96), o_inf = o_h + al(m * 32), total = o_inf + al(m);
    if (ctx->scr_in.reserve(total) || ctx->scr_status.reserve(m + 16)) return SSA_ERR_HIP;
    u8 *g = (u8 *)ctx->scr_in.p;
    int rc = timed_launch(ctx, "screen_gather", [&] {
        const unsigned gx = grid_for((size_t)pl.seg_lanes * 210u / 16u, 256u * 4u);
        hipLaunchKernelGGL(msm_k_screen_gather, dim3(gx, sl.count), dim3(256), 0, ctx->stream, sl, b.sigs, b.pks, b.pk_inf,
                           h, g, g + o_pks, g + o_inf, (u64 *)(g + o_h));
    });
    if (rc) return rc;
    const DevBatch gathered{g, g + o_pks, b.pk_inf ? g + o_inf : nullptr, {}};
    if ((rc = ssa_internal_verify_hashed(ctx, gathered, (const u64 *)(g + o_h), m, SSA_FLAG_SIG_FLAG_BYTE,
                                         (u8 *)ctx->scr_status.p, scratch_fail)))
        return rc;
    return timed_launch(ctx, "screen_scatter", [&] {
        hipLaunchKernelGGL(msm_k_screen_scatter, dim3(grid_for(m, 256)), dim3(256), 0, ctx->stream, sl, m,
                           (const u8 *)ctx->scr_status.p, d_status);
    });
}

static int screen_count(ssa_ctx *ctx, const uint8_t *d_status, size_t n, unsigned long long *d_fail) {
    HIP_TRY(hipMemsetAsync(d_fail, 0, sizeof(unsigned long long), ctx->stream));
    hipLaunchKernelGGL(msm_k_screen_count, dim3(grid_for(n, 256)), dim3(256), 0, ctx->stream, d_status, n, d_fail);
    HIP_TRY(hipGetLastError());
    return 0;
}

int ssa_internal_screen_hashed(ssa_ctx *ctx, const DevBatch &b, size_t n, const uint64_t *d_h, uint8_t *d_status,
                               unsigned long long *d_fail) {
    if (!d_h || !d_status || n == 0 || n > ctx->knobs.msm_slice) return SSA_ERR_ARG;
    if (int rc = screen_slice(ctx, b, n, nullptr, 0, (const u64 *)d_h, d_status)) return rc;
    return d_fail ? screen_count(ctx, d_status, n, d_fail) : 0;
}

extern "C" int ssa_verify_batch_screened_device(ssa_ctx *ctx, const uint8_t *d_sigs, const uint8_t *d_pks,
                                                const uint8_t *d_pk_inf, const uint8_t *d_msgs, const uint64_t *d_msg_off,
                                                size_t msg_stride, size_t msg_len, size_t n, const uint8_t *d_coeffs,
                                                uint32_t coeff_bytes, uint8_t *d_status_out, uint64_t *d_n_fail_out) {
    const DevBatch b{d_sigs, d_pks, d_pk_inf, {d_msgs, d_msg_off, msg_stride, msg_len}};
    if (int rc = check_dev_batch(ctx, b, n, d_status_out, d_coeffs, coeff_bytes)) return rc;
    unsigned long long *d_fail;
    if (int rc = reset_fail_counter(ctx, d_n_fail_out, &d_fail)) return rc;
    if (n == 0) return 0;
    if (n <= ctx->knobs.msm_small_max)
        return ssa_verify_many_device(ctx, d_sigs, d_pks, d_pk_inf, d_msgs, d_msg_off, msg_stride, msg_len, n,
                                      SSA_FLAG_SIG_FLAG_BYTE, d_status_out, (uint64_t *)d_fail);
    if (int rc = for_dev_slices(b, n, ctx->knobs.msm_slice, [&](size_t lo, size_t cnt, const DevBatch &s) {
            return screen_slice(ctx, s, cnt, d_coeffs ? d_coeffs + (size_t)coeff_bytes * lo : nullptr, coeff_bytes, nullptr,
                                d_status_out + lo);
        }))
        return rc;
    return screen_count(ctx, d_status_out, n, d_fail);
}

static int screen_host_one(ssa_ctx *ctx, const HostBatch &b, size_t n, const uint8_t *coeffs, uint8_t *status_out,
                           uint64_t *nf) {
    return status_host_one(ctx, b, n, coeffs, true, false, status_out, nf,
                           [&](const StagedInputs &s, u8 *d_status, unsigned long long *d_fail) {
        if (int r = screen_slice(ctx, s.batch, n, s.coeffs, 32, s.hashed ? (const u64 *)ctx->ws_h.p : nullptr, d_status))
            return r;
        return screen_count(ctx, d_status, n, d_fail);
    });
}

extern "C" int ssa_verify_batch_screened(ssa_ctx *ctx, const uint8_t *sigs, const uint8_t *pks, const uint8_t *pk_inf,
                                         const uint8_t *msgs, const uint64_t *msg_off, size_t msg_stride, size_t msg_len,
                                         size_t n, const uint8_t *coeffs, uint8_t *status_out, uint64_t *n_fail_out) {
    const HostBatch b{sigs, pks, pk_inf, msgs, msg_off, msg_stride, msg_len};
    if (int rc = check_host_batch(ctx, b, n, status_out)) return rc;
    if (n_fail_out) *n_fail_out = 0;
    if (n == 0) return 0;
    HIP_TRY(hipSetDevice(ctx->device));
    if (n <= ctx->knobs.msm_small_max)
        return ssa_verify_many(ctx, sigs, pks, pk_inf, msgs, msg_off, msg_stride, msg_len, n, SSA_FLAG_SIG_FLAG_BYTE,
                               status_out, n_fail_out);
    return run_host_slices_counted(ctx, b, n, ctx->knobs.msm_slice, n_fail_out,
                                   [&](ssa_ctx *c, size_t lo, size_t cnt, const HostBatch &s, uint64_t *nf) {
                                       return screen_host_one(c, s, cnt, coeffs ? coeffs + 32 * lo : nullptr,
                                                              status_out + lo, nf);
                                   });
}

constexpr uint32_t MANY_SCREEN_FLAGS = SSA_FLAG_CHECK_TORSION | SSA_FLAG_SIG_FLAG_BYTE;

static int screen_slice_after_keys(ssa_ctx *ctx, const DevBatch &b, size_t n, const uint8_t *d_coeffs, uint32_t coeff_bytes,
                                   uint32_t flags, const u64 *d_h, uint8_t *d_status, CallStats *stats, const KeyView &kv,
                                   uint64_t u, uint64_t hits, const unsigned long long *d_unpublished, uint64_t sv[12]);

static int screen_many_slice(ssa_ctx *ctx, const DevBatch &b, size_t n, const uint8_t *d_coeffs, uint32_t coeff_bytes,
                             uint32_t flags, const u64 *d_h, uint8_t *d_status, CallStats *stats, ssa_keycache *kc) {
    uint64_t sv[12] = {0, 0, 0, 0, 0, 0, 0, 0, 0, 0, 0, 0};
    if (ctx->scr_fail.reserve(16)) return SSA_ERR_HIP;
    unsigned long long *scratch_fail = (unsigned long long *)ctx->scr_fail.p;
    if (n <= ctx->knobs.msm_small_max) {
        sv[6] = 1;
        const int rc = d_h ? ssa_internal_verify_hashed(ctx, b, d_h, n, flags, d_status, scratch_fail)
                           : ssa_verify_many_device(ctx, b.sigs, b.pks, b.pk_inf, b.msgs.msgs, b.msgs.off, b.msgs.stride,
                                                    b.msgs.len, n, flags, d_status, (uint64_t *)scratch_fail);
        if (rc == 0 && stats) stats->add(sv);
        return rc;
    }
    uint64_t u = 0, hits = 0;
    KeyView kv{};
    const unsigned long long *d_unpublished = nullptr;
    if (kc) {
        if (int rc = ssa_internal_keycache_slice(ctx, kc, b.pks, b.pk_inf, n, &kv, &u, &hits, sv + 8, &d_unpublished)) return rc;
    } else {
        if (int rc = ssa_internal_dedup_keys(ctx, b.pks, b.pk_inf, n, &u, &hits)) return rc;
        kv = ctx_key_view(ctx, u);
    }
    return screen_slice_after_keys(ctx, b, n, d_coeffs, coeff_bytes, flags, d_h, d_status, stats, kv, u, hits, d_unpublished,
                                   sv);
}

static int screen_slice_after_keys(ssa_ctx *ctx, const DevBatch &b, size_t n, const uint8_t *d_coeffs, uint32_t coeff_bytes,
                                   uint32_t flags, const u64 *d_h, uint8_t *d_status, CallStats *stats, const KeyView &kv,
                                   uint64_t u, uint64_t hits, const unsigned long long *d_unpublished, uint64_t sv[12]) {
    unsigned long long *scratch_fail = (unsigned long long *)ctx->scr_fail.p;
    const unsigned nb = grid_for(n, SCR_BLOCK);
    if (ctx->scr_mask.reserve(n + 16) || ctx->scr_mark.reserve(n + 16) || ctx->scr_list.reserve(n * sizeof(u32)) ||
        ctx->scr_blk.reserve(2 * (size_t)nb * sizeof(u32)) || ctx->scr_cnt.reserve(64) || ctx->scr_ok.reserve(SCREEN_MAX_SEGS))
        return SSA_ERR_HIP;
    const u32 *key_idx = kv.lane_key;
    u8 *mark = (u8 *)ctx->scr_mark.p;
    u32 *blk_cnt = (u32 *)ctx->scr_blk.p, *blk_off = blk_cnt + nb, *list = (u32 *)ctx->scr_list.p;
    unsigned long long *d_cnt = (unsigned long long *)ctx->scr_cnt.p;
    int rc = timed_launch(ctx, "screen_keymask", [&] {
        hipLaunchKernelGGL(msm_k_screen_keymask, dim3(nb), dim3(SCR_BLOCK), 0, ctx->stream, key_idx,
                           kv.status, kv.n_keys, (u32)n, (u8 *)ctx->scr_mask.p);
    });
    if (rc) return rc;
    const ScreenPlan pl = screen_plan(n, ctx->knobs.screen_segs);
    ScreenArgs sa{pl.segs, pl.seg_lanes / 256u, d_status, (u8 *)ctx->scr_ok.p};
    sa.lane_mask = (const u8 *)ctx->scr_mask.p;
    sa.recheck = mark;
    if ((rc = msm_run_one(ctx, b, n, d_coeffs, coeff_bytes, nullptr, nullptr, d_h, &sa))) return rc;
    const u64 *h = d_h ? d_h : (const u64 *)ctx->ws_h.p;
    HIP_TRY(hipMemsetAsync(d_cnt, 0, 2 * sizeof(unsigned long long), ctx->stream));
    rc = timed_launch(ctx, "screen_mark", [&] {
        hipLaunchKernelGGL(msm_k_screen_mark, dim3(nb), dim3(SCR_BLOCK), 0, ctx->stream, (const u8 *)ctx->scr_ok.p,
                           pl.seg_lanes, (u32)n, mark, blk_cnt, d_cnt);
        hipLaunchKernelGGL(msm_k_screen_scan, dim3(1), dim3(SCR_BLOCK), 0, ctx->stream, (const u32 *)blk_cnt, (u32)nb,
                           blk_off, d_cnt);
    });
    if (rc) return rc;
    uint8_t ok[SCREEN_MAX_SEGS];
    unsigned long long cnt[2] = {0, 0}, unpublished = 0;
    HIP_TRY(hipMemcpyAsync(ok, ctx->scr_ok.p, pl.segs, hipMemcpyDeviceToHost, ctx->stream));
    HIP_TRY(hipMemcpyAsync(cnt, d_cnt, sizeof cnt, hipMemcpyDeviceToHost, ctx->stream));
    if (d_unpublished)
        HIP_TRY(hipMemcpyAsync(&unpublished, d_unpublished, sizeof unpublished, hipMemcpyDeviceToHost, ctx->stream));
    HIP_TRY(hipStreamSynchronize(ctx->stream));
    const size_t m = (size_t)cnt[1];
    if (m > n || cnt[0] > m) return SSA_ERR_HIP;
    sv[0] = u;
    sv[1] = pl.segs;
    for (u32 s = 0; s < pl.segs; s++) sv[2] += ok[s] ? 0 : 1;
    sv[3] = m;
    sv[4] = cnt[0];
    sv[5] = 1;
    sv[7] = hits + unpublished;
    if (m == 0) {
        if (stats) stats->add(sv);
        return 0;
    }
    if (2 * m > n) {
        sv[6] = 1;
        rc = ssa_internal_verify_keyed_view(ctx, b.sigs, key_idx, kv, h, n, flags, d_status, scratch_fail);
        if (rc == 0 && stats) stats->add(sv);
        return rc;
    }
    auto al = [](size_t b) { return (b + 255) & ~(size_t)255; };
    const size_t o_h = al(m * 81), o_idx = o_h + al(m * 32), total = o_idx + al(m * sizeof(u32));
    if (ctx->scr_in.reserve(total) || ctx->scr_status.reserve(m + 16)) return SSA_ERR_HIP;
    u8 *g = (u8 *)ctx->scr_in.p;
    rc = timed_launch(ctx, "screen_list_gather", [&] {
        hipLaunchKernelGGL(msm_k_screen_list, dim3(nb), dim3(SCR_BLOCK), 0, ctx->stream, (const u8 *)mark, (u32)n,
                           (const u32 *)blk_off, list);
        hipLaunchKernelGGL(msm_k_screen_gather_list, dim3(grid_for(m * 81, 256)), dim3(256), 0, ctx->stream,
                           (const u32 *)list, (u32)m, b.sigs, h, key_idx, g, (u64 *)(g + o_h), (u32 *)(g + o_idx));
    });
    if (rc) return rc;
    if ((rc = ssa_internal_verify_keyed_view(ctx, g, (const u32 *)(g + o_idx), kv, (const u64 *)(g + o_h), m, flags,
                                             (u8 *)ctx->scr_status.p, scratch_fail)))
        return rc;
    rc = timed_launch(ctx, "screen_list_scatter", [&] {
        hipLaunchKernelGGL(msm_k_screen_scatter_list, dim3(grid_for(m, 256)), dim3(256), 0, ctx->stream, (const u32 *)list,
                           (u32)m, (const u8 *)ctx->scr_status.p, d_status);
    });
    if (rc == 0 && stats) stats->add(sv);
    return rc;
}

static size_t many_screen_slice_lanes(const ssa_ctx *ctx) {
    const size_t cap = (size_t)1 << 23;
    return ctx->knobs.lane_slice < cap ? ctx->knobs.lane_slice : cap;
}

static int many_screened_device(ssa_ctx *ctx, ssa_keycache *kc, const DevBatch &b, size_t n, uint32_t flags,
                                const uint8_t *d_coeffs, uint32_t coeff_bytes, uint8_t *d_status_out, uint64_t *d_n_fail_out,
                                uint64_t *stats_out, int stats_words) {
    if (flags & ~MANY_SCREEN_FLAGS) return SSA_ERR_ARG;
    if (int rc = check_dev_batch(ctx, b, n, d_status_out, d_coeffs, coeff_bytes)) return rc;
    if (kc && (kc->ctx != ctx || kc->wire_mode)) return SSA_ERR_ARG;
    CallStats st(stats_words);
    st.out(stats_out);
    if (flags == SSA_FLAG_SIG_FLAG_BYTE)
        return ssa_verify_batch_screened_device(ctx, b.sigs, b.pks, b.pk_inf, b.msgs.msgs, b.msgs.off, b.msgs.stride,
                                                b.msgs.len, n, d_coeffs, coeff_bytes, d_status_out, d_n_fail_out);
    unsigned long long *d_fail;
    if (int rc = reset_fail_counter(ctx, d_n_fail_out, &d_fail)) return rc;
    if (n == 0) return 0;
    if (n <= ctx->knobs.msm_small_max) {
        const int rc = ssa_verify_many_device(ctx, b.sigs, b.pks, b.pk_inf, b.msgs.msgs, b.msgs.off, b.msgs.stride,
                                              b.msgs.len, n, flags, d_status_out, (uint64_t *)d_fail);
        if (rc == 0 && stats_out) stats_out[6] = 1;
        return rc;
    }
    if (int rc = for_dev_slices(b, n, many_screen_slice_lanes(ctx), [&](size_t lo, size_t cnt, const DevBatch &s) {
            return screen_many_slice(ctx, s, cnt, d_coeffs ? d_coeffs + (size_t)coeff_bytes * lo : nullptr, coeff_bytes,
                                     flags, nullptr, d_status_out + lo, stats_out ? &st : nullptr, kc);
        }))
        return rc;
    if (int rc = screen_count(ctx, d_status_out, n, d_fail)) return rc;
    st.out(stats_out);
    return 0;
}

extern "C" int ssa_verify_many_screened_device(ssa_ctx *ctx, const uint8_t *d_sigs, const uint8_t *d_pks,
                                               const uint8_t *d_pk_inf, const uint8_t *d_msgs, const uint64_t *d_msg_off,
                                               size_t msg_stride, size_t msg_len, size_t n, uint32_t flags,
                                               const uint8_t *d_coeffs, uint32_t coeff_bytes, uint8_t *d_status_out,
                                               uint64_t *d_n_fail_out, uint64_t stats_out[8]) {
    return many_screened_device(ctx, nullptr, {d_sigs, d_pks, d_pk_inf, {d_msgs, d_msg_off, msg_stride, msg_len}}, n, flags,
                                d_coeffs, coeff_bytes, d_status_out, d_n_fail_out, stats_out, 8);
}

static int screen_many_host_one(ssa_ctx *ctx, const HostBatch &b, size_t n, uint32_t flags, const uint8_t *coeffs,
                                uint8_t *status_out, uint64_t *nf, CallStats *stats, ssa_keycache *kc) {
    return status_host_one(ctx, b, n, coeffs, true, false, status_out, nf,
                           [&](const StagedInputs &s, u8 *d_status, unsigned long long *d_fail) {
        if (int r = screen_many_slice(ctx, s.batch, n, s.coeffs, 32, flags, s.hashed ? (const u64 *)ctx->ws_h.p : nullptr,
                                      d_status, stats, kc))
            return r;
        return screen_count(ctx, d_status, n, d_fail);
    });
}

template <class F>
static int host_slices_in_order(ssa_ctx *ctx, const HostBatch &b, size_t n, size_t slice, uint64_t *n_fail_out, F &&fn) {
    uint64_t total = 0;
    for (size_t lo = 0; lo < n; lo += slice) {
        const size_t cnt = n - lo < slice ? n - lo : slice;
        std::vector<uint64_t> off;
        uint64_t nf = 0;
        if (int rc = fn(ctx, lo, cnt, b.slice(lo, cnt, off), &nf)) return rc;
        total += nf;
    }
    if (n_fail_out) *n_fail_out = total;
    return 0;
}

static int many_screened_host(ssa_ctx *ctx, ssa_keycache *kc, const HostBatch &b, size_t n, uint32_t flags,
                              const uint8_t *coeffs, uint8_t *status_out, uint64_t *n_fail_out, uint64_t *stats_out,
                              int stats_words) {
    if (flags & ~MANY_SCREEN_FLAGS) return SSA_ERR_ARG;
    if (int rc = check_host_batch(ctx, b, n, status_out)) return rc;
    if (kc && (kc->ctx != ctx || kc->wire_mode)) return SSA_ERR_ARG;
    CallStats st(stats_words);
    st.out(stats_out);
    if (flags == SSA_FLAG_SIG_FLAG_BYTE)
        return ssa_verify_batch_screened(ctx, b.sigs, b.pks, b.pk_inf, b.msgs, b.msg_off, b.msg_stride, b.msg_len, n, coeffs,
                                         status_out, n_fail_out);
    if (n_fail_out) *n_fail_out = 0;
    if (n == 0) return 0;
    HIP_TRY(hipSetDevice(ctx->device));
    if (n <= ctx->knobs.msm_small_max) {
        const int rc = ssa_verify_many(ctx, b.sigs, b.pks, b.pk_inf, b.msgs, b.msg_off, b.msg_stride, b.msg_len, n, flags,
                                       status_out, n_fail_out);
        if (rc == 0 && stats_out) stats_out[6] = 1;
        return rc;
    }
    auto one = [&](ssa_ctx *c, size_t lo, size_t cnt, const HostBatch &s, uint64_t *nf) {
        return screen_many_host_one(c, s, cnt, flags, coeffs ? coeffs + 32 * lo : nullptr, status_out + lo, nf,
                                    stats_out ? &st : nullptr, kc);
    };
    const size_t slice = many_screen_slice_lanes(ctx);
    const int rc = kc ? host_slices_in_order(ctx, b, n, slice, n_fail_out, one)
                      : run_host_slices_counted(ctx, b, n, slice, n_fail_out, one);
    if (rc) return rc;
    st.out(stats_out);
    return 0;
}

extern "C" int ssa_verify_many_screened(ssa_ctx *ctx, const uint8_t *sigs, const uint8_t *pks, const uint8_t *pk_inf,
                                        const uint8_t *msgs, const uint64_t *msg_off, size_t msg_stride, size_t msg_len,
                                        size_t n, uint32_t flags, const uint8_t *coeffs, uint8_t *status_out,
                                        uint64_t *n_fail_out, uint64_t stats_out[8]) {
    return many_screened_host(ctx, nullptr, {sigs, pks, pk_inf, msgs, msg_off, msg_stride, msg_len}, n, flags, coeffs,
                              status_out, n_fail_out, stats_out, 8);
}

extern "C" int ssa_verify_many_cached_device(ssa_ctx *ctx, ssa_keycache *kc, const uint8_t *d_sigs, const uint8_t *d_pks,
                                             const uint8_t *d_pk_inf, const uint8_t *d_msgs, const uint64_t *d_msg_off,
                                             size_t msg_stride, size_t msg_len, size_t n, uint32_t flags,
                                             const uint8_t *d_coeffs, uint32_t coeff_bytes, uint8_t *d_status_out,
                                             uint64_t *d_n_fail_out, uint64_t stats_out[12]) {
    if (!kc) return SSA_ERR_ARG;
    return many_screened_device(ctx, kc, {d_sigs, d_pks, d_pk_inf, {d_msgs, d_msg_off, msg_stride, msg_len}}, n, flags,
                                d_coeffs, coeff_bytes, d_status_out, d_n_fail_out, stats_out, 12);
}

extern "C" int ssa_verify_many_cached(ssa_ctx *ctx, ssa_keycache *kc, const uint8_t *sigs, const uint8_t *pks,
                                      const uint8_t *pk_inf, const uint8_t *msgs, const uint64_t *msg_off, size_t msg_stride,
                                      size_t msg_len, size_t n, uint32_t flags, const uint8_t *coeffs, uint8_t *status_out,
                                      uint64_t *n_fail_out, uint64_t stats_out[12]) {
    if (!kc) return SSA_ERR_ARG;
    return many_screened_host(ctx, kc, {sigs, pks, pk_inf, msgs, msg_off, msg_stride, msg_len}, n, flags, coeffs, status_out,
                              n_fail_out, stats_out, 12);
}


struct SliceHash {
    u64 *h;
    u8 *dig;
};
static int keyed_hash_slice(ssa_ctx *ctx, const DevBatch &b, size_t n, const SliceHash &sh) {
    return ssa_internal_hash_scalars_digests(ctx, b, n, sh.h, sh.dig);
}

static int keyed_exact_slice(ssa_ctx *ctx, const uint8_t *d_keyed, const MsgView &mv, size_t n, uint32_t flags,
                             uint8_t *d_status, unsigned long long *d_fail, const SliceHash *sh = nullptr) {
    DevBatch b{nullptr, nullptr, nullptr, mv};
    if (int rc = ssa_internal_unpack_keyed(ctx, d_keyed, n, &b)) return rc;
    if (sh) {
        if (int rc = keyed_hash_slice(ctx, b, n, *sh)) return rc;
        return ssa_internal_verify_hashed(ctx, b, sh->h, n, flags, d_status, d_fail);
    }
    return ssa_verify_many_device(ctx, b.sigs, b.pks, b.pk_inf, mv.msgs, mv.off, mv.stride, mv.len, n, flags, d_status,
                                  (uint64_t *)d_fail);
}

static int check_keyed_dev(const ssa_ctx *ctx, const uint8_t *d_keyed, const MsgView &mv, size_t n,
                           const uint8_t *d_status_out, const uint8_t *d_coeffs, uint32_t coeff_bytes) {
    if (!ctx || (n && (!d_keyed || !d_status_out))) return SSA_ERR_ARG;
    if (d_coeffs && (coeff_bytes == 0 || coeff_bytes > 32)) return SSA_ERR_ARG;
    return check_msgs(mv, n);
}

extern "C" int ssa_verify_keyed_many_device(ssa_ctx *ctx, const uint8_t *d_keyed, const uint8_t *d_msgs,
                                            const uint64_t *d_msg_off, size_t msg_stride, size_t msg_len, size_t n,
                                            uint32_t flags, uint8_t *d_status_out, uint64_t *d_n_fail_out) {
    const MsgView mv{d_msgs, d_msg_off, msg_stride, msg_len};
    if (int rc = check_keyed_dev(ctx, d_keyed, mv, n, d_status_out, nullptr, 32)) return rc;
    unsigned long long *d_fail;
    if (int rc = reset_fail_counter(ctx, d_n_fail_out, &d_fail)) return rc;
    if (n == 0) return 0;
    if (n <= ctx->knobs.lane_slice) return keyed_exact_slice(ctx, d_keyed, mv, n, flags, d_status_out, d_fail);
    if (ctx->scr_fail.reserve(16)) return SSA_ERR_HIP;
    const DevBatch b{nullptr, nullptr, nullptr, mv};
    if (int rc = for_dev_slices(b, n, ctx->knobs.lane_slice, [&](size_t lo, size_t cnt, const DevBatch &s) {
            return keyed_exact_slice(ctx, d_keyed + 130 * lo, s.msgs, cnt, flags, d_status_out + lo,
                                     (unsigned long long *)ctx->scr_fail.p);
        }))
        return rc;
    return screen_count(ctx, d_status_out, n, d_fail);
}

static int keyed_cached_slice(ssa_ctx *ctx, ssa_keycache *kc, const uint8_t *d_keyed, const MsgView &mv, size_t n,
                              const uint8_t *d_coeffs, uint32_t coeff_bytes, uint32_t flags, uint8_t *d_status,
                              CallStats *stats, const SliceHash *sh = nullptr) {
    uint64_t sv[12] = {0, 0, 0, 0, 0, 0, 0, 0, 0, 0, 0, 0};
    if (ctx->scr_fail.reserve(16)) return SSA_ERR_HIP;
    if (n <= ctx->knobs.msm_small_max) {
        sv[6] = 1;
        const int rc = keyed_exact_slice(ctx, d_keyed, mv, n, flags, d_status, (unsigned long long *)ctx->scr_fail.p, sh);
        if (rc == 0 && stats) stats->add(sv);
        return rc;
    }
    uint64_t u = 0, hits = 0;
    KeyView kv{};
    DevBatch b{nullptr, nullptr, nullptr, mv};
    const unsigned long long *d_unpublished = nullptr;
    if (int rc = ssa_internal_keyed_cache_slice(ctx, kc, d_keyed, n, &b, &kv, &u, &hits, sv + 8, &d_unpublished)) return rc;
    if (sh) {
        if (int rc = keyed_hash_slice(ctx, b, n, *sh)) return rc;
        return screen_slice_after_keys(ctx, b, n, d_coeffs, coeff_bytes, flags, sh->h, d_status, stats, kv, u, hits,
                                       d_unpublished, sv);
    }
    return screen_slice_after_keys(ctx, b, n, d_coeffs, coeff_bytes, flags, nullptr, d_status, stats, kv, u, hits,
                                   d_unpublished, sv);
}

static int keyed_batch_screened_device(ssa_ctx *ctx, const uint8_t *d_keyed, const MsgView &mv, size_t n,
                                       const uint8_t *d_coeffs, uint32_t coeff_bytes, uint8_t *d_status_out,
                                       uint64_t *d_n_fail_out) {
    unsigned long long *d_fail;
    if (int rc = reset_fail_counter(ctx, d_n_fail_out, &d_fail)) return rc;
    if (n == 0) return 0;
    if (ctx->scr_fail.reserve(16)) return SSA_ERR_HIP;
    const DevBatch whole{nullptr, nullptr, nullptr, mv};
    if (int rc = for_dev_slices(whole, n, ctx->knobs.msm_slice, [&](size_t lo, size_t cnt, const DevBatch &s) {
            DevBatch b = s;
            if (int r = ssa_internal_unpack_keyed(ctx, d_keyed + 130 * lo, cnt, &b)) return r;
            return ssa_verify_batch_screened_device(ctx, b.sigs, b.pks, b.pk_inf, b.msgs.msgs, b.msgs.off, b.msgs.stride,
                                                    b.msgs.len, cnt, d_coeffs ? d_coeffs + (size_t)coeff_bytes * lo : nullptr,
                                                    coeff_bytes, d_status_out + lo, (uint64_t *)ctx->scr_fail.p);
        }))
        return rc;
    return screen_count(ctx, d_status_out, n, d_fail);
}

extern "C" int ssa_verify_keyed_many_cached_device(ssa_ctx *ctx, ssa_keycache *kc, const uint8_t *d_keyed,
                                                   const uint8_t *d_msgs, const uint64_t *d_msg_off, size_t msg_stride,
                                                   size_t msg_len, size_t n, uint32_t flags, const uint8_t *d_coeffs,
                                                   uint32_t coeff_bytes, uint8_t *d_status_out, uint64_t *d_n_fail_out,
                                                   uint64_t stats_out[12]) {
    if (flags & ~MANY_SCREEN_FLAGS) return SSA_ERR_ARG;
    if (!kc) return SSA_ERR_ARG;
    const MsgView mv{d_msgs, d_msg_off, msg_stride, msg_len};
    if (int rc = check_keyed_dev(ctx, d_keyed, mv, n, d_status_out, d_coeffs, coeff_bytes)) return rc;
    if (kc->ctx != ctx || !kc->wire_mode) return SSA_ERR_ARG;
    CallStats st(12);
// ... 118 lines not shown
```

Baseline: 30.55 million.

## Split large single-slice verify batches across twin stream for concurrent execution

When a batch fits in one lane slice and is large enough (default at least 2^19), it is split into a main part and a smaller fraction (default 2/16) that runs hash and verify on the twin context's stream, concurrently with the main part. The goal is to fill idle compute units during the main kernel's tail by overlapping a second kernel. The split only happens when this is the sole live context on the device, and internal callers are routed to a non-splitting path. The risk is contention between the two kernels and extra event synchronisation. Debug hooks for the split plan, config and timing are added as well.

```diff
diff --git a/include/schnorr_sig_amd.h b/include/schnorr_sig_amd.h
--- a/include/schnorr_sig_amd.h
+++ b/include/schnorr_sig_amd.h
@@ -499,6 +499,10 @@
 int ssa_debug_keytab_read(ssa_keyset *ks, ssa_keycache *kc, int what, uint64_t key, uint64_t *words_out);
 int ssa_debug_tail_plan(unsigned waves, unsigned pieces, unsigned gens, int uniform, unsigned min_main, size_t n,
                         uint32_t flags, uint32_t out[14]);
+int ssa_debug_split_plan(size_t n, uint32_t flags, size_t split_min, unsigned split_frac, size_t coop_max_n,
+                         size_t coop_max_n_torsion, int twin, uint64_t out[2]);
+int ssa_debug_split_config(ssa_ctx *ctx, int64_t split_min, int split_frac, int tail_b, int alone);
+int ssa_debug_split_timing(ssa_ctx *ctx, const char *kernel, double out[3]);
 int ssa_debug_screen_plan(size_t n, uint32_t coeff_bytes, uint64_t out[8]);
 int ssa_debug_screen_segments(ssa_ctx *ctx, uint32_t k);
 int ssa_debug_dedup_device(ssa_ctx *ctx, const uint8_t *d_pks, const uint8_t *d_pk_inf, size_t n,
diff --git a/schnorr-sig_amd/__init__.py b/schnorr-sig_amd/__init__.py
--- a/schnorr-sig_amd/__init__.py
+++ b/schnorr-sig_amd/__init__.py
@@ -164,6 +164,9 @@
         "ssa_ctx_stream_acquire": (i32, [vp, vp]),
         "ssa_debug_fault_after_chunk": (i32, [vp, i32]),
         "ssa_debug_tail_plan": (i32, [u32, u32, u32, i32, u32, sz, u32, vp]),
+        "ssa_debug_split_plan": (i32, [sz, u32, sz, u32, sz, sz, i32, vp]),
+        "ssa_debug_split_config": (i32, [vp, C.c_int64, i32, i32, i32]),
+        "ssa_debug_split_timing": (i32, [vp, C.c_char_p, vp]),
         "ssa_verify_batch_screened": (i32, [vp, vp, vp, vp, vp, vp, sz, sz, sz, vp, vp, u64p]),
         "ssa_verify_batch_screened_device": (i32, [vp, vp, vp, vp, vp, vp, sz, sz, sz, vp, u32, vp, vp]),
         "ssa_debug_screen_plan": (i32, [sz, u32, vp]),
@@ -1354,6 +1357,18 @@
                "ssa_ctx_read_timing")
         return avg.value, int(cnt.value)
 
+    def debug_split_config(self, split_min=-1, split_frac=-1, tail_b=-1, alone=-1):
+        _check(_lib.ssa_debug_split_config(self._ctx, int(split_min), int(split_frac), int(tail_b), int(alone)),
+               "ssa_debug_split_config")
+
+    def debug_split_timing(self, kernel):
+        out = np.zeros(3, dtype=np.float64)
+        rc = _lib.ssa_debug_split_timing(self._ctx, kernel.encode(), out.ctypes.data)
+        if rc == ERR_ARG:
+            return None
+        _check(rc, "ssa_debug_split_timing")
+        return tuple(float(v) for v in out)
+
     def host_path_probe(self, sigs_t, pks_t, msgs_t, n, reps=3):
         import time
         hs, hp, hm = (t[:n].cpu().numpy() for t in (sigs_t, pks_t, msgs_t))
@@ -2027,6 +2042,15 @@
         return (d & 1, bool(d & 2), bool(d & 4), (d >> 8) & 0xff, (d >> 16) & 0xff)
     return {"n_pieces": int(out[0]), "tail_groups": int(out[1]), "main_blocks": int(out[2]), "grid_blocks": int(out[3]),
             "pieces": [dec(out[4 + k]) for k in range(int(out[0]))], "whole": [dec(out[12]), dec(out[13])]}
+
+
+def debug_split_plan(n, split_frac, split_min=0, check_torsion=False, force_lane=False, coop_max_n=7680,
+                     coop_max_n_torsion=10496, twin=True):
+    out = np.zeros(2, dtype=np.uint64)
+    flags = (FLAG_CHECK_TORSION if check_torsion else 0) | (FLAG_FORCE_LANE if force_lane else 0)
+    _check(_lib.ssa_debug_split_plan(int(n), flags, int(split_min), int(split_frac), int(coop_max_n),
+                                     int(coop_max_n_torsion), int(bool(twin)), out.ctypes.data), "ssa_debug_split_plan")
+    return int(out[0]), int(out[1])
 
 
 def debug_screen_plan(n, coeff_bytes=0):
diff --git a/schnorr-sig_amd/csrc/ssa_api.hip b/schnorr-sig_amd/csrc/ssa_api.hip
--- a/schnorr-sig_amd/csrc/ssa_api.hip
+++ b/schnorr-sig_amd/csrc/ssa_api.hip
@@ -51,6 +51,17 @@
 };
 static std::mutex g_gtab_mu;
 static std::vector<SharedGtab *> g_gtabs;
+
+static std::mutex g_live_mu;
+static std::map<int, int> g_live_ctxs;
+static void live_ctxs_add(int device, int d) {
+    std::lock_guard<std::mutex> lock(g_live_mu);
+    g_live_ctxs[device] += d;
+}
+static int live_ctxs_on(int device) {
+    std::lock_guard<std::mutex> lock(g_live_mu);
+    return g_live_ctxs[device];
+}
 
 static inline size_t gtab_bytes(u32 bits) { return gtab_entries(bits) * 12 * sizeof(u64); }
 
@@ -190,6 +201,10 @@
     env_flag("SSA_MSM_OVERLAP", k.msm_overlap);
     env_int("SSA_PIPELINE_CHUNKS", 1, 8, k.pipeline_chunks);
     env_flag("SSA_TWO_STREAMS", ctx->two_streams);
+    env_u64("SSA_SPLIT_MIN", 0, UINT64_MAX, k.split_min);
+    env_int("SSA_SPLIT_FRAC", 0, 8, k.split_frac);
+    env_flag("SSA_SPLIT_TAIL_B", k.split_tail_b);
+    env_flag("SSA_SPLIT_ALONE", k.split_alone);
     uint64_t mb = 0;
     if (*hbm_budget_bytes == 0 && env_u64("SSA_HBM_BUDGET_MB", 0, UINT64_MAX, mb)) *hbm_budget_bytes = mb << 20;
     if (*gtab_bits == 0) env_one_of("SSA_GTAB_BITS", {16, 20, 22, 24}, *gtab_bits);
@@ -272,6 +287,10 @@
     HIP_TRY(hipMemcpyAsync(&gen_ok, ctx->ws_fail.p, sizeof gen_ok, hipMemcpyDeviceToHost, ctx->stream));
     HIP_TRY(hipStreamSynchronize(ctx->stream));
     if (gen_ok != 1u) return SSA_ERR_PARAMS;
+    if (!inherit) {
+        live_ctxs_add(device, 1);
+        ctx->counted_live = true;
+    }
     *out = guard.release();
     return 0;
 }
@@ -317,16 +336,14 @@
         ssa_ctx_destroy(ctx->twin);
         ctx->twin = nullptr;
     }
+    if (ctx->counted_live) live_ctxs_add(ctx->device, -1);
     orphan_handles(ctx->keysets, [](ssa_keyset *ks) { ks->release_all(); });
     orphan_handles(ctx->signer_sets, [](ssa_signer_set *ss) { ss->wipe_release(); });
     orphan_handles(ctx->keycaches, [](ssa_keycache *kc) { kc->release_all(); });
     orphan_handles(ctx->aggregators, [](ssa_aggregator *ag) { agx_release_all(*ag); });
     orphan_handles(ctx->aggverifiers, [](ssa_aggverifier *av) { agx_release_all(*av); });
     for (auto &kv : ctx->timed)
-        for (auto &t : kv.second) {
-            (void)hipEventDestroy(t.start);
-            (void)hipEventDestroy(t.stop);
-        }
+        for (auto &t : kv.second) timed_destroy(t);
     for_each_devbuf(ctx, [](DevBuf &b) { b.release(); });
     for_each_hostbuf(ctx, [](HostBuf &b) { b.release(); });
     if (ctx->d_params) (void)hipFree(ctx->d_params);
@@ -442,18 +459,36 @@
         if (it == c->timed.end()) continue;
         for (auto &t : it->second) {
             float ms = 0;
-            if (hipEventElapsedTime(&ms, t.start, t.stop) == hipSuccess) {
+            if (timed_ms(t, &ms)) {
                 total += ms;
                 cnt++;
             }
-            (void)hipEventDestroy(t.start);
-            (void)hipEventDestroy(t.stop);
+            timed_destroy(t);
         }
         c->timed.erase(it);
     }
     if (avg_ms) *avg_ms = cnt ? total / (double)cnt : 0.0;
     if (launches) *launches = cnt;
     return 0;
+}
+
+extern "C" int ssa_debug_split_timing(ssa_ctx *ctx, const char *kernel, double out[3]) {
+    if (!ctx || !kernel || !out) return SSA_ERR_ARG;
+    HIP_TRY(hipStreamSynchronize(ctx->stream));
+    const auto it = ctx->timed.find(kernel);
+    if (it == ctx->timed.end()) return SSA_ERR_ARG;
+    for (auto t = it->second.rbegin(); t != it->second.rend(); ++t) {
+        if (!t->start2) continue;
+        float span = 0, a = 0, b = 0;
+        if (!timed_ms(*t, &span)) return SSA_ERR_HIP;
+        HIP_TRY(hipEventElapsedTime(&a, t->start, t->stop));
+        HIP_TRY(hipEventElapsedTime(&b, t->start2, t->stop2));
+        out[0] = span;
+        out[1] = a;
+        out[2] = b;
+        return 0;
+    }
+    return SSA_ERR_ARG;
 }
 
 extern "C" int ssa_hash_message_many_device(ssa_ctx *ctx, const uint8_t *d_sigs, const uint8_t *d_pks,
@@ -582,23 +617,69 @@
     return 0;
 }
 
+struct SplitKnobs {
+    size_t min_n;
+    unsigned frac;
+    bool coop, twin;
+};
+static void split_plan_of(const SplitKnobs &kn, size_t n, size_t *nA, size_t *nB) {
+    *nA = n;
+    *nB = 0;
+    if (kn.frac == 0 || kn.frac > 8 || kn.coop || !kn.twin || n < kn.min_n) return;
+    const size_t want_b = n / 16 * kn.frac + n % 16 * kn.frac / 16;
+    const size_t a = (n - want_b + 255) / 256 * 256;
+    if (a >= n) return;
+    *nA = a;
+    *nB = n - a;
+}
+extern "C" int ssa_debug_split_plan(size_t n, uint32_t flags, size_t split_min, unsigned split_frac, size_t coop_max_n,
+                                    size_t coop_max_n_torsion, int twin, uint64_t out[2]) {
+    if (!out) return SSA_ERR_ARG;
+    size_t nA, nB;
+    split_plan_of({split_min, split_frac, takes_coop_of(coop_max_n, coop_max_n_torsion, n, flags), twin != 0}, n, &nA, &nB);
+    out[0] = nA;
+    out[1] = nB;
+    return 0;
+}
+extern "C" int ssa_debug_split_config(ssa_ctx *ctx, int64_t split_min, int split_frac, int tail_b, int alone) {
+    if (!ctx || split_frac > 8) return SSA_ERR_ARG;
+    if (alone >= 0) ctx->knobs.split_alone = alone != 0;
+    if (split_min >= 0) ctx->knobs.split_min = (size_t)split_min;
+    if (split_frac >= 0) ctx->knobs.split_frac = (unsigned)split_frac;
+    if (tail_b >= 0) ctx->knobs.split_tail_b = tail_b != 0;
+    return 0;
+}
+
+struct VerifyGrid {
+    TailPlan tp;
+    unsigned blocks;
+};
+static int verify_grid(ssa_ctx *c, size_t cnt, uint32_t flags, bool end_game, VerifyGrid *g) {
+    g->tp = end_game ? tail_plan(c, cnt, flags) : tail_plan_of({0u, 0u, 0u, c->knobs.verify_block, 0u, false, false}, cnt, flags);
+    g->blocks = grid_for(cnt, c->knobs.verify_block);
+    if (g->tp.n_pieces) {
+        if (c->tail_done.reserve(2 * (size_t)g->tp.tail_groups * sizeof(u32)) ||
+            c->tail_park.reserve((size_t)g->tp.tail_groups * PARK_WORDS * 64 * sizeof(u64)))
+            return SSA_ERR_HIP;
+        HIP_TRY(hipMemsetAsync(c->tail_done.p, 0, 2 * (size_t)g->tp.tail_groups * sizeof(u32), c->stream));
+        g->blocks = tail_grid_blocks(g->tp);
+    }
+    return 0;
+}
+static void verify_kernel(ssa_ctx *c, const VerifyGrid &g, const DevBatch &s, const u64 *d_h, u64 *d_tab, size_t cnt,
+                          uint32_t flags, uint8_t *d_status_out, unsigned long long *d_fail) {
+    hipLaunchKernelGGL(ssa_k_verify, dim3(g.blocks), dim3(c->knobs.verify_block), 0, c->stream, s.sigs, s.pks, s.pk_inf, d_h,
+                       (const u64 *)c->d_gtab, d_tab, cnt, flags, d_status_out, d_fail, g.tp, (u32 *)c->tail_done.p,
+                       (u64 *)c->tail_park.p);
+}
+
 static int verify_slices(ssa_ctx *ctx, const DevBatch &b, const u64 *d_h, size_t n, uint32_t flags, uint8_t *d_status_out,
                          unsigned long long *d_fail) {
     return for_dev_slices(b, n, ctx->knobs.lane_slice, [&](size_t lo, size_t cnt, const DevBatch &s) {
-        const TailPlan tp = tail_plan(ctx, cnt, flags);
-        unsigned blocks = grid_for(cnt, ctx->knobs.verify_block);
-        if (tp.n_pieces) {
-            if (ctx->tail_done.reserve(2 * (size_t)tp.tail_groups * sizeof(u32)) ||
-                ctx->tail_park.reserve((size_t)tp.tail_groups * PARK_WORDS * 64 * sizeof(u64)))
-                return SSA_ERR_HIP;
-            HIP_TRY(hipMemsetAsync(ctx->tail_done.p, 0, 2 * (size_t)tp.tail_groups * sizeof(u32), ctx->stream));
-            blocks = tail_grid_blocks(tp);
-        }
+        VerifyGrid g;
+        if (int rc = verify_grid(ctx, cnt, flags, true, &g)) return rc;
         return timed_launch(ctx, "ssa_k_verify", [&] {
-            hipLaunchKernelGGL(ssa_k_verify, dim3(blocks), dim3(ctx->knobs.verify_block), 0,
-                               ctx->stream, s.sigs, s.pks, s.pk_inf, d_h + 4 * lo, (const u64 *)ctx->d_gtab,
-                               (u64 *)ctx->ws_tab.p, cnt, flags, d_status_out + lo, d_fail, tp, (u32 *)ctx->tail_done.p,
-                               (u64 *)ctx->tail_park.p);
+            verify_kernel(ctx, g, s, d_h + 4 * lo, (u64 *)ctx->ws_tab.p, cnt, flags, d_status_out + lo, d_fail);
         });
     });
 }
@@ -622,8 +703,56 @@
     return verify_slices(c, b, (const u64 *)c->ws_h.p, cnt, flags, d_status_out, d_fail);
 }
 
+static int verify_split(ssa_ctx *ctx, ssa_ctx *tw, const DevBatch &b, size_t nA, size_t nB, uint32_t flags,
+                        uint8_t *d_status_out, unsigned long long *d_fail) {
+    constexpr size_t TAB_WORDS = (size_t)(PTAB_ENTRIES * PTAB_ENTRY_U64);
+    const size_t n = nA + nB;
+    if (ctx->ws_h.reserve(n * 4 * sizeof(u64)) || ctx->ws_tab.reserve(n * TAB_WORDS * sizeof(u64))) return SSA_ERR_HIP;
+    u64 *h = (u64 *)ctx->ws_h.p, *tab = (u64 *)ctx->ws_tab.p;
+    const DevBatch bB = b.slice(nA);
+    HIP_TRY(hipEventRecord(ctx->order_ev, ctx->stream));
+    HIP_TRY(hipStreamWaitEvent(tw->stream, ctx->order_ev, 0));
+    TimedLaunch th{}, tv{};
+    const bool timing = ctx->knobs.timing;
+    auto mark = [&](hipEvent_t *ev, hipStream_t st) {
+        if (!timing) return 0;
+        HIP_TRY(hipEventCreate(ev));
+        HIP_TRY(hipEventRecord(*ev, st));
+        return 0;
+    };
+    auto hash = [&](ssa_ctx *c, const DevBatch &s, size_t cnt, u64 *d_h, hipEvent_t *start, hipEvent_t *stop) {
+        if (int r = mark(start, c->stream)) return r;
+        hipLaunchKernelGGL(ssa_k_hash, dim3(grid_for(cnt, 256)), dim3(256), 0, c->stream, c->d_params, s.sigs, s.pks, s.msgs,
+                           cnt, d_h, (u8 *)nullptr, (const u32 *)nullptr, 0u);
+        HIP_TRY(hipGetLastError());
+        return mark(stop, c->stream);
+    };
+    auto verify = [&](ssa_ctx *c, const DevBatch &s, size_t lo, size_t cnt, bool end_game, hipEvent_t *start, hipEvent_t *stop) {
+        VerifyGrid g;
+        if (int r = verify_grid(c, cnt, flags, end_game, &g)) return r;
+        if (int r = mark(start, c->stream)) return r;
+        verify_kernel(c, g, s, h + 4 * lo, tab + lo * TAB_WORDS, cnt, flags, d_status_out + lo, d_fail);
+        HIP_TRY(hipGetLastError());
+        return mark(stop, c->stream);
+    };
+    int rc = hash(ctx, b, nA, h, &th.start, &th.stop);
+    if (rc == 0) rc = hash(tw, bB, nB, h + 4 * nA, &th.start2, &th.stop2);
+    if (rc == 0) rc = verify(tw, bB, nA, nB, ctx->knobs.split_tail_b, &tv.start2, &tv.stop2);
+    if (rc == 0) rc = verify(ctx, b, 0, nA, true, &tv.start, &tv.stop);
+    if (timing && rc == 0) {
+        ctx->timed["ssa_k_hash"].push_back(th);
+        ctx->timed["ssa_k_verify"].push_back(tv);
+    } else {
+        timed_destroy(th);
+        timed_destroy(tv);
+    }
+    if (hipEventRecord(tw->order_ev, tw->stream) != hipSuccess || hipStreamWaitEvent(ctx->stream, tw->order_ev, 0) != hipSuccess)
+        return rc ? rc : SSA_ERR_HIP;
+    return rc;
+}
+
 static int verify_launch(ssa_ctx *ctx, const DevBatch &b, size_t n, uint32_t flags, uint8_t *d_status_out,
-                         unsigned long long *d_fail) {
+                         unsigned long long *d_fail, bool may_split = false) {
     if (takes_coop(ctx, n, flags)) {
         return timed_launch(ctx, "ssa_k_verify_coop", [&] {
             hipLaunchKernelGGL(ssa_k_verify_coop, dim3((unsigned)n), dim3(128), 0, ctx->stream, ctx->d_params, b.sigs,
@@ -631,7 +760,15 @@
         });
     }
     const size_t slice = ctx->knobs.lane_slice < n ? ctx->knobs.lane_slice : n;
-    if (n <= slice) return verify_one_slice(ctx, b, n, flags, d_status_out, d_fail);
+    if (n <= slice) {
+        if (may_split && ctx->knobs.split_frac && n >= ctx->knobs.split_min && (!ctx->knobs.split_alone || live_ctxs_on(ctx->device) == 1)) {
+            ssa_ctx *tw = ssa_internal_twin(ctx);
+            size_t nA, nB;
+            split_plan_of({ctx->knobs.split_min, ctx->knobs.split_frac, false, tw != nullptr}, n, &nA, &nB);
+            if (nB) return verify_split(ctx, tw, b, nA, nB, flags, d_status_out, d_fail);
+        }
+        return verify_one_slice(ctx, b, n, flags, d_status_out, d_fail);
+    }
     ssa_ctx *tw = ssa_internal_twin(ctx);
     if (tw) {
         HIP_TRY(hipEventRecord(ctx->order_ev, ctx->stream));
@@ -652,17 +789,29 @@
     return rc;
 }
 
+static int verify_many_device(ssa_ctx *ctx, const DevBatch &b, size_t n, uint32_t flags, uint8_t *d_status_out,
+                              uint64_t *d_n_fail_out, bool may_split) {
+    if (int rc = check_dev_batch(ctx, b, n, d_status_out)) return rc;
+    unsigned long long *d_fail;
+    if (int rc = reset_fail_counter(ctx, d_n_fail_out, &d_fail)) return rc;
+    if (n == 0) return 0;
+    return verify_launch(ctx, b, n, flags, d_status_out, d_fail, may_split);
+}
+
 extern "C" int ssa_verify_many_device(ssa_ctx *ctx, const uint8_t *d_sigs, const uint8_t *d_pks,
                                       const uint8_t *d_pk_inf, const uint8_t *d_msgs,
                                       const uint64_t *d_msg_off, size_t msg_stride, size_t msg_len,
                                       size_t n, uint32_t flags, uint8_t *d_status_out,
                                       uint64_t *d_n_fail_out) {
-    const DevBatch b{d_sigs, d_pks, d_pk_inf, {d_msgs, d_msg_off, msg_stride, msg_len}};
-    if (int rc = check_dev_batch(ctx, b, n, d_status_out)) return rc;
-    unsigned long long *d_fail;
-    if (int rc = reset_fail_counter(ctx, d_n_fail_out, &d_fail)) return rc;
-    if (n == 0) return 0;
-    return verify_launch(ctx, b, n, flags, d_status_out, d_fail);
+    return verify_many_device(ctx, {d_sigs, d_pks, d_pk_inf, {d_msgs, d_msg_off, msg_stride, msg_len}}, n, flags,
+                              d_status_out, d_n_fail_out, true);
+}
+
+int ssa_internal_verify_many_device(ssa_ctx *ctx, const uint8_t *d_sigs, const uint8_t *d_pks, const uint8_t *d_pk_inf,
+                                    const uint8_t *d_msgs, const uint64_t *d_msg_off, size_t msg_stride, size_t msg_len,
+                                    size_t n, uint32_t flags, uint8_t *d_status_out, uint64_t *d_n_fail_out) {
+    return verify_many_device(ctx, {d_sigs, d_pks, d_pk_inf, {d_msgs, d_msg_off, msg_stride, msg_len}}, n, flags,
+                              d_status_out, d_n_fail_out, false);
 }
 
 int ssa_internal_sign_vartime(ssa_ctx *ctx, const uint8_t *d_sks, const uint8_t *d_nonces, const MsgView &mv, size_t n,
@@ -814,8 +963,8 @@
     unsigned long long nf = 0, *d_fail = (unsigned long long *)ctx->ws_fail.p;
     hc.copy_back(&nf, d_fail, sizeof nf);
     if (int rc = hc.finish([&] {
-            return ssa_verify_many_device(ctx, d_sigs, d_pks, d_inf, mv.msgs, mv.off, b.msg_stride, b.msg_len, n, flags,
-                                          d_status, (uint64_t *)d_fail);
+            return ssa_internal_verify_many_device(ctx, d_sigs, d_pks, d_inf, mv.msgs, mv.off, b.msg_stride, b.msg_len, n, flags,
+                                                   d_status, (uint64_t *)d_fail);
         }))
         return rc;
     if (n_fail_out) *n_fail_out = nf;
diff --git a/schnorr-sig_amd/csrc/ssa_ctx.hpp b/schnorr-sig_amd/csrc/ssa_ctx.hpp
--- a/schnorr-sig_amd/csrc/ssa_ctx.hpp
+++ b/schnorr-sig_amd/csrc/ssa_ctx.hpp
@@ -89,6 +89,7 @@
 
 struct TimedLaunch {
     hipEvent_t start, stop;
+    hipEvent_t start2 = nullptr, stop2 = nullptr;
 };
 
 constexpr double DEDUP_RATIO_NO_CHECK = 0.0, DEDUP_RATIO_CHECK = 1.0;
@@ -112,6 +113,10 @@
     unsigned tail_min_main = 0;
     unsigned tail_waves_override = 0;
     bool timing = false;
+    size_t split_min = (size_t)1 << 19;
+    unsigned split_frac = 2;
+    bool split_tail_b = false;
+    bool split_alone = true;
     unsigned screen_segs = 0;
     double dedup_ratio[2] = {DEDUP_RATIO_NO_CHECK, DEDUP_RATIO_CHECK};
     unsigned dedup_probe_bound = DEDUP_PROBE_BOUND;
@@ -190,6 +195,7 @@
     DevParams h_params;
     ssa_ctx *twin = nullptr;
     bool is_twin = false, two_streams = true;
+    bool counted_live = false;
 #define X(name) DevBuf name;
     SSA_CTX_DEVBUFS(X)
 #undef X
@@ -305,6 +311,22 @@
     return 0;
 }
 
+static inline bool timed_ms(const TimedLaunch &t, float *ms) {
+    if (hipEventElapsedTime(ms, t.start, t.stop) != hipSuccess) return false;
+    if (!t.start2) return true;
+    for (hipEvent_t s : {t.start, t.start2})
+        for (hipEvent_t e : {t.stop, t.stop2}) {
+            float d = 0;
+            if (hipEventElapsedTime(&d, s, e) != hipSuccess) return false;
+            if (d > *ms) *ms = d;
+        }
+    return true;
+}
+static inline void timed_destroy(TimedLaunch &t) {
+    for (hipEvent_t ev : {t.start, t.stop, t.start2, t.stop2})
+        if (ev) (void)hipEventDestroy(ev);
+}
+
 
 static inline int check_msgs(const MsgView &mv, size_t n) {
     if (n == 0) return 0;
@@ -382,9 +404,12 @@
     return check_msgs(b.msgs, n);
 }
 
+static inline bool takes_coop_of(size_t coop_max_n, size_t coop_max_n_torsion, size_t n, uint32_t flags) {
+    const size_t coop_lim = (flags & SSA_FLAG_CHECK_TORSION) ? coop_max_n_torsion : coop_max_n;
+    return (flags & SSA_FLAG_FORCE_COOP) || (!(flags & SSA_FLAG_FORCE_LANE) && n <= coop_lim);
+}
 static inline bool takes_coop(const ssa_ctx *ctx, size_t n, uint32_t flags) {
-    const size_t coop_lim = (flags & SSA_FLAG_CHECK_TORSION) ? ctx->knobs.coop_max_n_torsion : ctx->knobs.coop_max_n;
-    return (flags & SSA_FLAG_FORCE_COOP) || (!(flags & SSA_FLAG_FORCE_LANE) && n <= coop_lim);
+    return takes_coop_of(ctx->knobs.coop_max_n, ctx->knobs.coop_max_n_torsion, n, flags);
 }
 
 struct CallStats {
@@ -709,6 +734,10 @@
 int ssa_internal_verify_hashed(ssa_ctx *ctx, const DevBatch &b, const uint64_t *d_h, size_t n, uint32_t flags,
                                uint8_t *d_status_out, unsigned long long *d_fail);
 
+int ssa_internal_verify_many_device(ssa_ctx *ctx, const uint8_t *d_sigs, const uint8_t *d_pks, const uint8_t *d_pk_inf,
+                                    const uint8_t *d_msgs, const uint64_t *d_msg_off, size_t msg_stride, size_t msg_len,
+                                    size_t n, uint32_t flags, uint8_t *d_status_out, uint64_t *d_n_fail_out);
+
 int ssa_internal_dedup_keys(ssa_ctx *ctx, const uint8_t *d_pks, const uint8_t *d_pk_inf, size_t cnt, uint64_t *u_out,
                             uint64_t *bound_hits_out);
 int ssa_internal_verify_keyed(ssa_ctx *ctx, const uint8_t *d_sigs, const uint32_t *d_key_idx, uint64_t u,
diff --git a/schnorr-sig_amd/csrc/ssa_msm.hip b/schnorr-sig_amd/csrc/ssa_msm.hip
--- a/schnorr-sig_amd/csrc/ssa_msm.hip
+++ b/schnorr-sig_amd/csrc/ssa_msm.hip
@@ -1437,8 +1437,8 @@
     unsigned long long *scratch_fail = (unsigned long long *)ctx->scr_fail.p;
     if (n <= ctx->knobs.msm_small_max) {
         if (d_h) return ssa_internal_verify_hashed(ctx, b, d_h, n, SSA_FLAG_SIG_FLAG_BYTE, d_status, scratch_fail);
-        return ssa_verify_many_device(ctx, b.sigs, b.pks, b.pk_inf, b.msgs.msgs, b.msgs.off, b.msgs.stride, b.msgs.len, n,
-                                      SSA_FLAG_SIG_FLAG_BYTE, d_status, (uint64_t *)scratch_fail);
+        return ssa_internal_verify_many_device(ctx, b.sigs, b.pks, b.pk_inf, b.msgs.msgs, b.msgs.off, b.msgs.stride, b.msgs.len, n,
+                                               SSA_FLAG_SIG_FLAG_BYTE, d_status, (uint64_t *)scratch_fail);
     }
     const ScreenPlan pl = screen_plan(n, ctx->knobs.screen_segs);
     if (ctx->scr_ok.reserve(SCREEN_MAX_SEGS)) return SSA_ERR_HIP;
@@ -1505,8 +1505,8 @@
     if (int rc = reset_fail_counter(ctx, d_n_fail_out, &d_fail)) return rc;
     if (n == 0) return 0;
     if (n <= ctx->knobs.msm_small_max)
-        return ssa_verify_many_device(ctx, d_sigs, d_pks, d_pk_inf, d_msgs, d_msg_off, msg_stride, msg_len, n,
-                                      SSA_FLAG_SIG_FLAG_BYTE, d_status_out, (uint64_t *)d_fail);
+        return ssa_internal_verify_many_device(ctx, d_sigs, d_pks, d_pk_inf, d_msgs, d_msg_off, msg_stride, msg_len, n,
+                                               SSA_FLAG_SIG_FLAG_BYTE, d_status_out, (uint64_t *)d_fail);
     if (int rc = for_dev_slices(b, n, ctx->knobs.msm_slice, [&](size_t lo, size_t cnt, const DevBatch &s) {
             return screen_slice(ctx, s, cnt, d_coeffs ? d_coeffs + (size_t)coeff_bytes * lo : nullptr, coeff_bytes, nullptr,
                                 d_status_out + lo);
@@ -1557,8 +1557,8 @@
     if (n <= ctx->knobs.msm_small_max) {
         sv[6] = 1;
         const int rc = d_h ? ssa_internal_verify_hashed(ctx, b, d_h, n, flags, d_status, scratch_fail)
-                           : ssa_verify_many_device(ctx, b.sigs, b.pks, b.pk_inf, b.msgs.msgs, b.msgs.off, b.msgs.stride,
-                                                    b.msgs.len, n, flags, d_status, (uint64_t *)scratch_fail);
+                           : ssa_internal_verify_many_device(ctx, b.sigs, b.pks, b.pk_inf, b.msgs.msgs, b.msgs.off, b.msgs.stride,
+                                                             b.msgs.len, n, flags, d_status, (uint64_t *)scratch_fail);
         if (rc == 0 && stats) stats->add(sv);
         return rc;
     }
@@ -1674,8 +1674,8 @@
     if (int rc = reset_fail_counter(ctx, d_n_fail_out, &d_fail)) return rc;
     if (n == 0) return 0;
     if (n <= ctx->knobs.msm_small_max) {
-        const int rc = ssa_verify_many_device(ctx, b.sigs, b.pks, b.pk_inf, b.msgs.msgs, b.msgs.off, b.msgs.stride,
-                                              b.msgs.len, n, flags, d_status_out, (uint64_t *)d_fail);
+        const int rc = ssa_internal_verify_many_device(ctx, b.sigs, b.pks, b.pk_inf, b.msgs.msgs, b.msgs.off, b.msgs.stride,
+                                                       b.msgs.len, n, flags, d_status_out, (uint64_t *)d_fail);
         if (rc == 0 && stats_out) stats_out[6] = 1;
         return rc;
     }
@@ -1799,8 +1799,8 @@
         if (int rc = keyed_hash_slice(ctx, b, n, *sh)) return rc;
         return ssa_internal_verify_hashed(ctx, b, sh->h, n, flags, d_status, d_fail);
     }
-    return ssa_verify_many_device(ctx, b.sigs, b.pks, b.pk_inf, mv.msgs, mv.off, mv.stride, mv.len, n, flags, d_status,
-                                  (uint64_t *)d_fail);
+    return ssa_internal_verify_many_device(ctx, b.sigs, b.pks, b.pk_inf, mv.msgs, mv.off, mv.stride, mv.len, n, flags, d_status,
+                                           (uint64_t *)d_fail);
 }
 
 static int check_keyed_dev(const ssa_ctx *ctx, const uint8_t *d_keyed, const MsgView &mv, size_t n,
```

After: 30.92 million (median of 6 runs). 1.01x the previous value.
